# LPD-EPFL-ML/X-MAP

Hardware: AMD Instinct MI355X
Metric: item_sim_pairs_per_s (higher is better)
Workload: dtype f64

## Files before the change

include/xmap_hip.h:

```cpp
#ifndef XMAP_HIP_H
#define XMAP_HIP_H
#include <stdint.h>

#ifdef __cplusplus
extern "C" {
#endif

#define XMAP_OK 0
#define XMAP_ERR_HIP -1
#define XMAP_ERR_ARG -2
#define XMAP_ERR_OVERFLOW -3
#define XMAP_ERR_CAPACITY -4

#define XMAP_COSINE 0
#define XMAP_ADJUST_COSINE 1
#define XMAP_COSINE_EXACT 2

#define XMAP_TOPC 10

typedef struct xmap_ratings {
    int64_t n_users;
    int32_t n_items;
    int64_t nnz;
    const int64_t *user_ptr;
    const int32_t *user_item;
    const float *user_rating;
    const int64_t *user_time;
    const int64_t *item_ptr;
    const int32_t *item_user;
    const float *item_rating;
    const int32_t *prefix_cls;
    const int32_t *suffix_cls;
    const uint32_t *contains_mask;
    const uint8_t *flags;
} xmap_ratings;

const char *xmap_last_error(void);
int xmap_version(void);

int xmap_trim(void);
int xmap_debug_arena(void *stream, int64_t *live, int64_t *reserved);
int xmap_debug_arena_call(void *stream, int64_t bytes, int fail);

int xmap_exclusive_scan_i64(void *stream, const int64_t *in, int64_t *out, int64_t n, int64_t *h_total);
int xmap_exclusive_scan_i32_to_i64(void *stream, const int32_t *in, int64_t *out, int64_t n, int64_t *h_total);


int xmap_build_csc(void *stream, int64_t n_users, int32_t n_items, int64_t nnz, const int64_t *user_ptr,
                   const int32_t *user_item, const float *user_rating, int32_t *cnt ,
                   int64_t *item_ptr , int32_t *item_user , float *item_rating );

int xmap_user_stats(void *stream, const xmap_ratings *R, double *u_avg, double *u_norm2);

int xmap_item_stats(void *stream, const xmap_ratings *R, const double *u_avg, double *info ,
                    double *norms ,
                    int32_t *ua_item , int32_t *ia_user ,
                    int32_t item_lo, int32_t item_hi );

#ifdef XMAP_CROSSCHECK
int xmap_sim_plan(void *stream, const xmap_ratings *R, int32_t slot_target, int32_t *Q, int64_t *W, int64_t *unit_ptr,
                  int64_t *h_n_units, int64_t *h_contrib);
int xmap_sim_units(void *stream, int32_t n_items, const int32_t *Q, const int64_t *unit_ptr,
                   int32_t *unit_item , int32_t *unit_q );

int xmap_sim_count(void *stream, const xmap_ratings *R, int method, int cap, const double *u_avg,
                   const double *info, const int32_t *ua_item, const int32_t *ia_user, const int32_t *Q,
                   const int32_t *unit_item, const int32_t *unit_q, int64_t unit_lo, int64_t unit_hi,
                   int32_t *unit_cnt , int64_t *d_counters , int64_t *h_counters );
int xmap_sim_fill(void *stream, const xmap_ratings *R, int method, int cap, const double *u_avg,
                  const double *info, const int32_t *ua_item, const int32_t *ia_user, const int32_t *Q,
                  const int32_t *unit_item, const int32_t *unit_q, int64_t unit_lo, int64_t unit_hi,
                  const int64_t *unit_off , int32_t *col, double *sim, int32_t *mutu, int32_t *nij);

int xmap_sim_row_ptr(void *stream, int32_t n_items, const int64_t *unit_ptr, const int64_t *unit_off ,
                     int64_t *row_ptr );
#endif

int xmap_sim2_layout(void *stream, const xmap_ratings *R, const double *info, int32_t ch_min, int32_t *hist ,
                     int64_t *pre , int32_t *ctl , int32_t *hid , int32_t *hlist ,
                     uint64_t *ub_key , void *ub ,
                     void *rc ,
                     uint64_t *Wp ,
                     int32_t dups , int32_t *h_ctl );
int xmap_sim2_plan(void *stream, const xmap_ratings *R, int32_t slot_target, const void *rc, const int64_t *pre,
                   const int32_t *hid, const int32_t *ctl, int32_t *Q, int32_t *C, uint8_t *small ,
                   uint64_t *Wp , int32_t *Qcat , int64_t *uq_ptr ,
                   int64_t *uc_ptr , int32_t dups, int64_t *h_counts );
int xmap_sim2_units(void *stream, int32_t n_items, const int64_t *item_ptr, const int32_t *Qcat, const int64_t *uq_ptr,
                    int32_t *uq_item, int32_t *uq_q , const int32_t *C, const int64_t *uc_ptr, int32_t *uc_item,
                    int32_t *uc_c);
int xmap_sim2_pairs(void *stream, const xmap_ratings *R, int method, int cap, const double *u_avg, const double *norms,
                    const void *rc, const void *ub, const int32_t *Q,
                    const uint8_t *small, const int32_t *uq_item, const int32_t *uq_q, const int64_t *cls_ptr ,
                    int64_t unit_lo, int64_t unit_hi, const int32_t *hid,
                    const int32_t *hlist, const int32_t *ctl, const int32_t *C, const int64_t *uc_ptr,
                    const int32_t *uc_item, const int32_t *uc_c, int32_t n_heavy_units, int32_t n_heavy, int phases,
                    double *hp_hi, double *hp_lo, int32_t *hp_cnt, int32_t *hp_mut, int64_t coo_cap, int32_t *coo_i,
                    int32_t *coo_j, double *coo_sim, int32_t *coo_mutu, int32_t *coo_nij,
                    double *coo_ls , int32_t *rowcnt,
                    int32_t *rowcnt_h , int64_t *d_shards ,
                    int64_t *d_counters ,
                    int32_t *mircnt );
int xmap_sim2_scatter(void *stream, int32_t n_items, int64_t n_coo, const int32_t *coo_i, const int32_t *coo_j,
                      const double *coo_sim, const int32_t *coo_mutu, const int32_t *coo_nij, const double *coo_ls ,
                      const int64_t *row_ptr, int32_t *fill , const int32_t *hid, const int32_t *hlist,
                      int32_t *col, double *sim, int32_t *mutu, int32_t *nij, double *ls );
int xmap_sim3_layout(void *stream, const xmap_ratings *R, int64_t *item_ptr ,
                     const double *rating64 , int32_t ch_min, int32_t phases, int32_t stats_lo, int32_t stats_hi,
                     int32_t *cnt ,
                     double *u_avg , double *u_norm , int32_t *hist ,
                     int64_t *pre , int32_t *ctl , int32_t *hid , int32_t *hlist ,
                     uint64_t *ub_key , void *ub , void *srec ,
                     void *bufA , void *bufB , void *rc ,
                     uint64_t *Wp , double *info , double *norms , int32_t *h_ctl );
int xmap_sim3_plan(void *stream, const xmap_ratings *R, int32_t slot_target, const int64_t *pre, const int32_t *hid,
                   const int32_t *ctl, int32_t *Q, int32_t *C, uint8_t *small, uint64_t *Wp, int32_t *Qcat ,
                   int64_t *uq_ptr , int64_t *uc_ptr , int32_t dups, int32_t *uq_item, int32_t *uq_q ,
                   int32_t *uc_item, int32_t *uc_c, int64_t cap_light, int64_t cap_heavy, int64_t *h_out );
int xmap_sim3_mircount(void *stream, int32_t n_items, int64_t coo_cap, const int32_t *coo_i, const int32_t *coo_j,
                       const int64_t *d_shards , int64_t n_pairs, int32_t skip_self, void *scratch, int32_t *mir );
int xmap_sim3_mirror(void *stream, int32_t n_items, int64_t coo_cap, const int32_t *coo_i, const int32_t *coo_j,
                     const double *coo_sim, const int32_t *coo_mutu, const int32_t *coo_nij,
                     const int64_t *d_shards ,
                     int64_t n_pairs, const int32_t *own , const int32_t *mir , int32_t *tot ,
                     int64_t *row_ptr , int64_t *mptr , int32_t *fill ,
                     void *bufA , void *bufB , int32_t *col,
                     double *sim, int32_t *mutu, int32_t *nij, const double *coo_aux , double *aux ,
                     int32_t row_lo, int32_t row_hi );

int xmap_sim2_pack_pairs(void *stream, int64_t n_coo, const int32_t *coo_i, const int32_t *coo_j, const double *coo_sim,
                         const int32_t *coo_mutu, const int32_t *coo_nij, int64_t *rec , int64_t *h_count);
int xmap_sim2_unpack_pairs(void *stream, int64_t n, const int64_t *rec , int32_t *coo_i, int32_t *coo_j, double *coo_sim,
                           int32_t *coo_mutu, int32_t *coo_nij);
int xmap_item_partials(void *stream, const xmap_ratings *R, const double *u_avg, double *partial );
int xmap_item_merge(void *stream, int32_t n_items, int32_t n_parts, const double *parts , double *info ,
                    double *norms );
int xmap_sim2_pack_partials(void *stream, int64_t n_coo, const int32_t *coo_i, const int32_t *coo_j, const double *coo_hi,
                            const double *coo_lo, const int32_t *coo_mutu, const int32_t *coo_nij, int64_t *rec ,
                            int64_t *h_count);
int xmap_sim2_sort_partials(void *stream, int64_t n, const int64_t *rec , int64_t *rec_sorted , int32_t n_items,
                            int32_t n_owners );
int xmap_sim2_merge_partials(void *stream, int method, int cap, int32_t n_items, int64_t n, const int64_t *rec_sorted,
                             const double *norms , int32_t *coo_i, int32_t *coo_j, double *coo_sim, int32_t *coo_mutu,
                             int32_t *coo_nij, int32_t *rowcnt , int64_t *h_counts );



typedef struct xmap_sim {
    int32_t n_items;
    const int64_t *row_ptr;
    const int32_t *col;
    const double *sim;
    const int32_t *mutu;
    const int32_t *nij;
    const double *info;
    const double *frac;
} xmap_sim;

int xmap_bridge_flags(void *stream, const xmap_sim *S, const int32_t *prefix_cls, uint8_t *bb);

int xmap_knn_classify(void *stream, const xmap_sim *S, int top_k, const uint8_t *bb, const int32_t *suffix_cls,
                      const uint32_t *contains_mask, uint8_t *cls, int32_t *kcnt ,
                      int32_t *kcol , double *kval ,
                      int32_t row_lo, int32_t row_hi );

int xmap_knn_thresholds(void *stream, int32_t n_items, int top_k, const int32_t *kcnt, const int32_t *kcol, const double *kval,
                        void *thr );
int xmap_reverse_count(void *stream, const xmap_sim *S, int mode, int top_k, const uint8_t *bb, const uint8_t *cls,
                       const int32_t *kcnt, const int32_t *kcol, const double *kval, const int32_t *suffix_cls,
// ... 112 lines not shown
int xmap_rec_select(void *stream, int32_t n_items, const int64_t *row_ptr, const int32_t *col, const double *sim,
                    const double *ls, int32_t keep, int32_t *out_cnt, int32_t *out_col, double *out_sim, double *out_ls);

int xmap_predict(void *stream, int64_t n_test, const int32_t *test_user, const int32_t *test_item, const int64_t *nb_ptr,
                 const int32_t *nb_item, const double *nb_sim, const int64_t *rt_ptr, const int32_t *rt_user, const double *rt_rating,
                 const double *rt_time, const double *item_avg, const double *wtab, int32_t n_w, double *out_plain,
                 double *out_decay, int32_t *status);

int xmap_rec_profiles(void *stream, int64_t n_users, int64_t n_rows, int64_t n_target_rows, const int64_t *off_t, const int64_t *off_m,
                      const int32_t *user, const int32_t *item, const double *rating, const int64_t *time, int64_t *prof_ptr,
                      int32_t *prof_item, double *prof_rating, int64_t *prof_time);
int xmap_predict_rows(void *stream, int64_t n_test, const int32_t *test_user, const int32_t *test_item, int64_t n_users,
                      int32_t n_items, int32_t keep, const int32_t *nb_cnt, const int32_t *nb_col, const double *nb_sim,
                      const int64_t *prof_ptr, const int32_t *prof_item, const double *prof_rating, const int64_t *prof_time,
                      const double *item_avg, const double *wtab, int32_t n_w, double *out_plain, double *out_decay,
                      int32_t *status, int32_t *h_max_now);
int xmap_mae(void *stream, int64_t n_test, const int32_t *status, const double *real, const double *out_plain, const double *out_decay,
             double *mae );


int xmap_select_map(void *stream, int32_t n_items, int private_flag, const int32_t *n_cand, const int32_t *top_end,
                    const int32_t *picks , int32_t *n_top, int32_t *choice, int32_t *map_src2tgt);

int xmap_alterego_count(void *stream, const xmap_ratings *R, const int32_t *map_src2tgt, int32_t *cnt_t, int32_t *cnt_m,
                        int64_t *d_profiles );
int xmap_alterego_fill(void *stream, const xmap_ratings *R, const int32_t *map_src2tgt, const int64_t *off_t,
                       const int64_t *off_m, int64_t n_t_total, int32_t *out_user, int32_t *out_item,
                       double *out_rating, int64_t *out_time);

typedef struct xmap_ctx xmap_ctx;

typedef struct xmap_feed xmap_feed;
int xmap_feed_text(const char *text, int64_t len, int32_t year_from, int32_t year_to, const char *label, int32_t min_ratings,
                   xmap_feed **out);
int xmap_feed_texts(int32_t n_parts, const char *const *texts, const int64_t *lens, const char *const *labels, int32_t year_from,
                    int32_t year_to, int32_t min_ratings, xmap_feed **out);
int xmap_feed_merge(const xmap_feed *a, const xmap_feed *b, xmap_feed **out);
int xmap_feed_sizes(const xmap_feed *f, int64_t *sizes );
int xmap_feed_arrays(const xmap_feed *f, int64_t *user_ptr, int32_t *item, double *rating, double *when, int32_t *prefix_cls,
                     int32_t *suffix_cls, uint32_t *contains_mask, uint8_t *flags);
int xmap_feed_ids(const xmap_feed *f, int32_t which, char *bytes, int64_t *offsets);
void xmap_feed_free(xmap_feed *f);
int xmap_ctx_upload_feed(xmap_ctx *ctx, const xmap_feed *f);
int xmap_feed_format(int64_t n_users, const int64_t *user_ptr, const int32_t *item, const float *rating, const int64_t *when,
                     const char *uid_fmt, const char *iid_fmt, const int64_t *item_number, int32_t item_lo, int32_t item_hi,
                     char *out, int64_t cap, int64_t *written);

int xmap_ctx_create(int device, xmap_ctx **out);
void xmap_ctx_destroy(xmap_ctx *ctx);
int xmap_ctx_upload_ratings(xmap_ctx *ctx, int64_t n_users, int32_t n_items, const int64_t *user_ptr, const int32_t *item,
                            const float *rating, const int64_t *time, const int32_t *prefix_cls, const int32_t *suffix_cls,
                            const uint32_t *contains_mask, const uint8_t *flags);
int xmap_ctx_item_sim(xmap_ctx *ctx, int method, int cap, int64_t *n_kept, int64_t *n_evaluated);
int xmap_ctx_sim_download(xmap_ctx *ctx, int64_t *row_ptr, int32_t *col, double *sim, int32_t *mutu, int32_t *nij, double *info,
                          double *user_avg);
int xmap_ctx_extend(xmap_ctx *ctx, int top_k, int64_t *n_out, int64_t *n_paths);
int xmap_ctx_ext_download(xmap_ctx *ctx, int32_t *n_cand, int32_t *top_end, double *top_val);
int xmap_ctx_ext_lists(xmap_ctx *ctx, int64_t *xs_off, int32_t *xs_end, double *xs_val);
int xmap_ctx_candidates(xmap_ctx *ctx, int32_t *n_top);
int xmap_ctx_generate(xmap_ctx *ctx, int private_flag, const int32_t *picks, int32_t *choice, int64_t *n_rows,
                      int64_t *n_target_rows);
int xmap_ctx_gen_download(xmap_ctx *ctx, int32_t *user, int32_t *item, double *rating, int64_t *time);
int xmap_ctx_rec_sim(xmap_ctx *ctx, int cap, int64_t *n_pairs);
int xmap_ctx_rec_profiles_download(xmap_ctx *ctx, int64_t *prof_ptr, int32_t *prof_item, double *prof_rating, int64_t *prof_time);
int xmap_ctx_rec_download(xmap_ctx *ctx, int64_t *row_ptr, int32_t *col, double *sim, double *ls, int32_t *nij, double *item_avg,
                          double *item_norm);
int xmap_ctx_rec_select(xmap_ctx *ctx, int keep);
int xmap_ctx_rec_set_neighbors(xmap_ctx *ctx, int keep, const int32_t *cnt, const int32_t *col, const double *sim);
int xmap_ctx_rec_neighbors_download(xmap_ctx *ctx, int32_t *cnt, int32_t *col, double *sim, double *ls);
int xmap_ctx_predict(xmap_ctx *ctx, int64_t n_test, const int32_t *test_user, const int32_t *test_item, const double *test_rating,
                     const double *wtab, int32_t n_w, double *out_plain, double *out_decay, int32_t *status, double *mae,
                     int32_t *max_now);

#ifdef __cplusplus
}
#endif
#endif
```

profiles/lds_atomic.hip:

```cpp
#include <hip/hip_runtime.h>
#include <stdio.h>
#define CK(x) do { hipError_t e_ = (x); if (e_ != hipSuccess) { printf("%s -> %s\n", #x, hipGetErrorString(e_)); return 1; } } while (0)
__device__ __forceinline__ unsigned long long mix(unsigned long long z) {
    z += 0x9E3779B97F4A7C15ull; z = (z ^ (z >> 30)) * 0xBF58476D1CE4E5B9ull; z = (z ^ (z >> 27)) * 0x94D049BB133111EBull;
    return z ^ (z >> 31);
}
template <int MODE>
__global__ __launch_bounds__(1024) void k(double *out, int steps, int n_slots) {
    extern __shared__ double tab[];
    for (int i = threadIdx.x; i < n_slots * 4; i += 1024) tab[i] = 0.0;
    __syncthreads();
    unsigned long long s = mix(blockIdx.x * 1024ull + threadIdx.x);
    double chk = 0.0;
    for (int it = 0; it < steps; it++) {
        s = mix(s);
        const int slot = (int)(s % (unsigned)n_slots);
        const double v = (double)(s & 1023) * 0.001, c = 0.5;
        double *a = tab + slot * 4;
        if (MODE == 0) {
            const double o = atomicAdd(a, v);
            const double sum = o + v, bb = sum - o;
            const double err = (o - (sum - bb)) + (v - bb);
            atomicAdd(a + 1, err);
            const double o2 = atomicAdd(a + 2, c);
            const double sum2 = o2 + c, bb2 = sum2 - o2;
            const double err2 = (o2 - (sum2 - bb2)) + (c - bb2);
            atomicAdd(a + 3, err2);
        } else {
            double h = a[0], l = a[1], h2 = a[2], l2 = a[3];
            double sum = h + v, bb = sum - h; double e = (h - (sum - bb)) + (v - bb); e += l; double hh = sum + e; l = e - (hh - sum); h = hh;
            double sum2 = h2 + c, bb2 = sum2 - h2; double e2 = (h2 - (sum2 - bb2)) + (c - bb2); e2 += l2; double hh2 = sum2 + e2; l2 = e2 - (hh2 - sum2); h2 = hh2;
            a[0] = h; a[1] = l; a[2] = h2; a[3] = l2;
        }
    }
    __syncthreads();
    for (int i = threadIdx.x; i < n_slots * 4; i += 1024) chk += tab[i];
    if (chk == 12345.678) out[0] = chk;
}
int main() {
    double *out; CK(hipMalloc(&out, 8));
    hipEvent_t e0, e1; CK(hipEventCreate(&e0)); CK(hipEventCreate(&e1));
    const int steps = 4096, blocks = 256 * 4;
    for (int n_slots : {512, 2048, 4096}) {
        const size_t lds = (size_t)n_slots * 32;
        CK(hipFuncSetAttribute((const void *)k<0>, hipFuncAttributeMaxDynamicSharedMemorySize, (int)lds));
        CK(hipFuncSetAttribute((const void *)k<1>, hipFuncAttributeMaxDynamicSharedMemorySize, (int)lds));
        for (int mode = 0; mode < 2; mode++)
            for (int rep = 0; rep < 2; rep++) {
                CK(hipEventRecord(e0));
                if (mode == 0) k<0><<<blocks, 1024, lds>>>(out, steps, n_slots); else k<1><<<blocks, 1024, lds>>>(out, steps, n_slots);
                CK(hipEventRecord(e1)); CK(hipEventSynchronize(e1));
                float ms; CK(hipEventElapsedTime(&ms, e0, e1));
                const double n = (double)blocks * 1024 * steps;
                if (rep) printf("slots %5d mode %d (%s): %7.2f ms  %.3e updates/s\n", n_slots, mode, mode ? "plain 32-B RMW" : "4 atomics + 2 two-sums", ms, n / (ms * 1e-3));
            }
    }
    return 0;
}
```

x-map_amd/csrc/api.hip:

```cpp
#include <math.h>
#include <stdlib.h>
#include <vector>

#include "common.h"

namespace xmap {

struct Pool {
    std::vector<void *> ptrs;
    void release() {
        for (void *p : ptrs) (void)hipFree(p);
        ptrs.clear();
    }
};

}

using namespace xmap;

struct xmap_ctx {
    int device = 0;
    hipStream_t st = nullptr;
    Pool p_ratings, p_sim, p_ext, p_gen, p_rows;
    xmap_ratings R;
    bool have_ratings = false;
    bool plain_exact = true;
    bool have_sim = false;
    xmap_sim S;
    double *u_avg = nullptr, *u_norm = nullptr, *info = nullptr;
    int64_t n_kept = 0, n_eval = 0, n_contrib = 0;
    int64_t half_contrib = 0;
    bool have_ext = false;
    int top_k = 0;
    xmap_ext_tables T;
    xmap_path_units Un;
    int32_t *n_cand = nullptr, *top_end = nullptr;
    double *top_val = nullptr;
    int64_t n_out = 0, n_paths = 0;
    double *acc = nullptr, *hacc = nullptr;
    int32_t *touched = nullptr, *htouched = nullptr;
    int64_t acc_slots = 0, acc_len = 0, hacc_rows = 0, hacc_len = 0;
    int32_t n_slots = 0;
    int32_t fast_div = 0;
    bool have_gen = false;
    int32_t *g_user = nullptr, *g_item = nullptr;
    double *g_rating = nullptr;
    int64_t *g_time = nullptr;
    int64_t n_rows = 0, n_target_rows = 0;
    int64_t *g_off_t = nullptr, *g_off_m = nullptr;
    Pool p_rec, p_nb;
    bool have_rec = false, have_nb = false;
    int64_t *pf_ptr = nullptr, *pf_time = nullptr;
    int32_t *pf_item = nullptr;
    double *pf_rating = nullptr;
    int64_t *rs_row_ptr = nullptr;
    int32_t *rs_col = nullptr, *rs_nij = nullptr;
    double *rs_sim = nullptr, *rs_ls = nullptr, *rs_avg = nullptr, *rs_norm = nullptr;
    int64_t rec_pairs = 0;
    int keep = 0;
    int32_t *nb_cnt = nullptr, *nb_col = nullptr;
    double *nb_sim = nullptr, *nb_ls = nullptr;
};

namespace xmap {

template <typename T>
static int dalloc(Pool &pool, T **out, size_t n, hipStream_t st, bool zero = false) {
    void *p = nullptr;
    const size_t bytes = sizeof(T) * (n ? n : 1);
    XM_HIP(hipMalloc(&p, bytes));
    pool.ptrs.push_back(p);
    if (zero) XM_HIP(hipMemsetAsync(p, 0, bytes, st));
    *out = (T *)p;
    return XMAP_OK;
}
#define XM_TRY(call) do { int rc_ = (call); if (rc_) return rc_; } while (0)
#define XM_ALLOC(pool, ptr, n) XM_TRY(dalloc(pool, &(ptr), (size_t)(n), c->st))
#define XM_ALLOCZ(pool, ptr, n) XM_TRY(dalloc(pool, &(ptr), (size_t)(n), c->st, true))

// ... 148 lines not shown
    R.n_users = n_users; R.n_items = n_items; R.nnz = nnz;
    c->half_contrib = 0;
    for (int64_t u = 0; u < n_users; u++) { const int64_t d = user_ptr[u + 1] - user_ptr[u]; c->half_contrib += d * (d - 1) / 2; }
    int64_t *d_ptr, *d_time, *d_iptr;
    int32_t *d_item, *d_iuser, *d_pre, *d_suf;
    float *d_rating, *d_irating;
    uint32_t *d_mask;
    uint8_t *d_flags;
    XM_TRY(h2d(c->p_ratings, &d_ptr, user_ptr, (size_t)n_users + 1, c->st));
    XM_TRY(h2d(c->p_ratings, &d_item, item, (size_t)nnz, c->st));
    XM_TRY(h2d(c->p_ratings, &d_rating, rating, (size_t)nnz, c->st));
    XM_TRY(h2d(c->p_ratings, &d_time, time, (size_t)nnz, c->st));
    XM_TRY(h2d(c->p_ratings, &d_pre, prefix_cls, (size_t)n_items, c->st));
    XM_TRY(h2d(c->p_ratings, &d_suf, suffix_cls, (size_t)n_items, c->st));
    XM_TRY(h2d(c->p_ratings, &d_mask, contains_mask, (size_t)n_items, c->st));
    XM_TRY(h2d(c->p_ratings, &d_flags, flags, (size_t)n_items, c->st));
    XM_ALLOCZ(c->p_ratings, d_iptr, n_items + 1);
    XM_ALLOCZ(c->p_ratings, d_iuser, nnz);
    XM_ALLOCZ(c->p_ratings, d_irating, nnz);
    R.user_ptr = d_ptr; R.user_item = d_item; R.user_rating = d_rating; R.user_time = d_time;
    R.item_ptr = d_iptr; R.item_user = d_iuser; R.item_rating = d_irating;
    R.prefix_cls = d_pre; R.suffix_cls = d_suf; R.contains_mask = d_mask; R.flags = d_flags;
    c->plain_exact = plain_sums_exact(n_users, nnz, rating);
    XM_HIP(hipStreamSynchronize(c->st));
    c->have_ratings = true;
    return XMAP_OK;
}

int xmap_ctx_item_sim(xmap_ctx *c, int method, int cap, int64_t *n_kept, int64_t *n_evaluated) {
    XM_ARG(c && c->have_ratings && (method == XMAP_COSINE || method == XMAP_ADJUST_COSINE) && cap > 0);
    XM_HIP(hipSetDevice(c->device));
    drop_tail(c);
    c->p_gen.release(); c->p_ext.release(); c->p_sim.release();
    c->have_sim = c->have_ext = c->have_gen = false;
    xmap_ratings &R = c->R;
    const int I = R.n_items;
    const int64_t U = R.n_users, nnz = R.nnz;
    const int pair_method = (method == XMAP_COSINE && !c->plain_exact) ? XMAP_COSINE_EXACT : method;
    Pool tmp;
    struct Guard { Pool &p; ~Guard() { p.release(); } } guard{tmp};
#define T_ALLOC(ptr, n) XM_TRY(dalloc(tmp, &(ptr), (size_t)(n), c->st))
#define T_ALLOCZ(ptr, n) XM_TRY(dalloc(tmp, &(ptr), (size_t)(n), c->st, true))
    int32_t *cnt;
    T_ALLOC(cnt, I);
    double *norms;
    XM_ALLOC(c->p_sim, c->u_avg, U);
    XM_ALLOC(c->p_sim, c->u_norm, U);
    XM_ALLOCZ(c->p_sim, c->info, (size_t)I * 4);
    T_ALLOCZ(norms, (size_t)2 * I);
    int32_t *hist, *ctl, *hid, *hlist;
    int64_t *pre;
    uint64_t *ub_key, *ub, *rcrec, *Wp, *srec, *buf_a, *buf_b;
    const size_t n1 = (size_t)(nnz ? nnz : 1);
    T_ALLOC(hist, U + 2); T_ALLOC(pre, U + 3); T_ALLOC(ctl, 4); T_ALLOC(hid, I); T_ALLOCZ(hlist, 1024);
    T_ALLOC(ub_key, n1); T_ALLOC(ub, n1); T_ALLOC(rcrec, 2 * n1); T_ALLOC(Wp, I);
    T_ALLOC(srec, 2 * n1); T_ALLOC(buf_a, 2 * n1); T_ALLOC(buf_b, 2 * n1);
    const int ch_min = 2048;
    XM_TRY(xmap_sim3_layout(c->st, &R, (int64_t *)R.item_ptr, nullptr, ch_min, 1 | 2 | 4, 0, I, cnt, c->u_avg, c->u_norm, hist, pre, ctl,
                            hid, hlist, ub_key, ub, srec, buf_a, buf_b, rcrec, Wp, c->info, norms, nullptr));
    const int64_t half_contrib = c->half_contrib;
    int32_t *Q, *Cc, *Qcat, *uq_item = nullptr, *uq_q = nullptr, *uc_item = nullptr, *uc_c = nullptr;
    uint8_t *small;
    int64_t *uq_ptr, *uc_ptr;
    T_ALLOCZ(Q, I); T_ALLOCZ(Cc, I); T_ALLOCZ(small, I); T_ALLOC(Qcat, (size_t)5 * (I ? I : 1)); T_ALLOCZ(uq_ptr, (size_t)5 * I + 1);
    T_ALLOCZ(uc_ptr, I + 1);
    int slot_target = 768;
    double coo_slack = 1.0;
    int64_t hc[10];
    int64_t n_light = 0, n_hu = 0;
    int n_heavy = 0;
    auto plan = [&](int target) -> int {
        const int64_t cap_light = half_contrib / target + I + 1, cap_heavy = nnz / ch_min + 1025;
        T_ALLOC(uq_item, cap_light); T_ALLOC(uq_q, 4 * cap_light); T_ALLOC(uc_item, cap_heavy); T_ALLOC(uc_c, cap_heavy);
        XM_TRY(xmap_sim3_plan(c->st, &R, target, pre, hid, ctl, Q, Cc, small, Wp, Qcat, uq_ptr, uc_ptr, 0, uq_item, uq_q, uc_item, uc_c,
                              cap_light, cap_heavy, hc));
        n_light = hc[0]; n_hu = hc[1]; n_heavy = (int)hc[9];
        return XMAP_OK;
    };
    XM_TRY(plan(slot_target));
    int32_t *coo_i = nullptr, *coo_j = nullptr, *coo_mutu = nullptr, *coo_nij = nullptr, *own = nullptr, *mir = nullptr;
    double *coo_sim = nullptr;
    int64_t *d_shards = nullptr;
    int64_t cap_coo = 0, n = 0, n_unordered = 0;
    for (;;) {
        cap_coo = ((int64_t)((double)(half_contrib > 0 ? half_contrib : 1) * coo_slack) / 4096 + 1100) * 4096;
        double *hp_hi, *hp_lo;
        int32_t *hp_cnt, *hp_mut, *rowcnt_h;
        int64_t *d_cnt;
        T_ALLOC(coo_i, cap_coo); T_ALLOC(coo_j, cap_coo); T_ALLOC(coo_sim, cap_coo); T_ALLOC(coo_mutu, cap_coo); T_ALLOC(coo_nij, cap_coo);
        T_ALLOC(own, I); T_ALLOC(mir, I);
        const size_t hp = (size_t)(n_hu ? n_hu : 1) * 1024;
        T_ALLOC(hp_hi, hp); T_ALLOC(hp_lo, hp); T_ALLOC(hp_cnt, hp); T_ALLOC(hp_mut, hp);
        T_ALLOCZ(d_cnt, 6); T_ALLOC(d_shards, 2 * 4096); T_ALLOC(rowcnt_h, 64 * 1024);
        XM_TRY(xmap_sim2_pairs(c->st, &R, pair_method, cap, c->u_avg, norms, rcrec, ub, Q, small, uq_item, uq_q, hc + 2, 0, n_light, hid, hlist,
                               ctl, Cc, uc_ptr, uc_item, uc_c, (int32_t)n_hu, n_heavy, 8 | 1 | 2 | 4 | 16 | 64 | 128, hp_hi, hp_lo, hp_cnt,
                               hp_mut, cap_coo, coo_i, coo_j, coo_sim, coo_mutu, coo_nij, nullptr, own, rowcnt_h, d_shards, d_cnt, mir));
        int64_t h_cnt[6];
        XM_TRY(d2h(h_cnt, d_cnt, 6, c->st));
        XM_HIP(hipStreamSynchronize(c->st));
        if (h_cnt[2]) {
            if (slot_target <= 32) { set_error("pair-table overflow"); return XMAP_ERR_OVERFLOW; }
            slot_target /= 2;
            XM_TRY(plan(slot_target));
            continue;
        }
        if (h_cnt[3]) {
            if (coo_slack > 64) { set_error("half-COO overflow"); return XMAP_ERR_CAPACITY; }
            coo_slack *= 2;
            continue;
        }
        n = h_cnt[4]; n_unordered = h_cnt[5];
        break;
    }
    int64_t *row_ptr, *mptr;
    XM_ALLOCZ(c->p_sim, row_ptr, I + 1);
    T_ALLOCZ(mptr, I + 1);
    const int64_t kept = 2 * n;
    int32_t *col, *mutu, *nij, *fill, *tot;
    double *sim;
    uint64_t *mir_a, *mir_b;
    XM_ALLOC(c->p_sim, col, kept); XM_ALLOC(c->p_sim, sim, kept); XM_ALLOC(c->p_sim, mutu, kept); XM_ALLOC(c->p_sim, nij, kept);
    T_ALLOC(fill, I); T_ALLOC(tot, I); T_ALLOC(mir_a, (size_t)3 * (n ? n : 1)); T_ALLOC(mir_b, (size_t)3 * (n ? n : 1));
    XM_TRY(xmap_sim3_mircount(c->st, I, cap_coo, coo_i, coo_j, d_shards, n, 0, mir_a, mir));
    XM_TRY(xmap_sim3_mirror(c->st, I, cap_coo, coo_i, coo_j, coo_sim, coo_mutu, coo_nij, d_shards, n, own, mir, tot, row_ptr, mptr, fill,
                            mir_a, mir_b, col, sim, mutu, nij, nullptr, nullptr, 0, I));
    XM_HIP(hipStreamSynchronize(c->st));
    c->S.n_items = I; c->S.row_ptr = row_ptr; c->S.col = col; c->S.sim = sim; c->S.mutu = mutu; c->S.nij = nij; c->S.info = c->info;
    c->S.frac = nullptr;
    c->n_kept = kept; c->n_eval = 2 * n_unordered; c->n_contrib = 2 * half_contrib;
    c->have_sim = true;
    if (n_kept) *n_kept = kept;
    if (n_evaluated) *n_evaluated = c->n_eval;
    return XMAP_OK;
#undef T_ALLOC
#undef T_ALLOCZ
}

int xmap_ctx_sim_download(xmap_ctx *c, int64_t *row_ptr, int32_t *col, double *sim, int32_t *mutu, int32_t *nij, double *info,
                          double *user_avg) {
    XM_ARG(c && c->have_sim);
    XM_HIP(hipSetDevice(c->device));
    const int I = c->R.n_items;
    if (row_ptr) XM_TRY(d2h(row_ptr, c->S.row_ptr, (size_t)I + 1, c->st));
    if (col) XM_TRY(d2h(col, c->S.col, (size_t)c->n_kept, c->st));
    if (sim) XM_TRY(d2h(sim, c->S.sim, (size_t)c->n_kept, c->st));
    if (mutu) XM_TRY(d2h(mutu, c->S.mutu, (size_t)c->n_kept, c->st));
    if (nij) XM_TRY(d2h(nij, c->S.nij, (size_t)c->n_kept, c->st));
    if (info) XM_TRY(d2h(info, (const double *)c->info, (size_t)I * 4, c->st));
    if (user_avg) XM_TRY(d2h(user_avg, (const double *)c->u_avg, (size_t)c->R.n_users, c->st));
    XM_HIP(hipStreamSynchronize(c->st));
    return XMAP_OK;
}

int xmap_ctx_extend(xmap_ctx *c, int top_k, int64_t *n_out, int64_t *n_paths) {
    XM_ARG(c && c->have_sim && top_k >= 1);
    XM_HIP(hipSetDevice(c->device));
    drop_tail(c);
    c->p_gen.release(); c->p_ext.release();
    c->have_ext = c->have_gen = false;
    const int I = c->R.n_items, k = top_k;
    c->top_k = k;
    xmap_ext_tables &T = c->T;
    memset(&T, 0, sizeof(T));
    T.n_items = I; T.top_k = k; T.flags = c->R.flags;
    XM_ALLOCZ(c->p_ext, c->n_cand, I);
    XM_ALLOC(c->p_ext, c->top_end, (size_t)I * XMAP_TOPC);
    XM_ALLOCZ(c->p_ext, c->top_val, (size_t)I * XMAP_TOPC);
    c->n_out = c->n_paths = 0;
    if (I == 0) { c->have_ext = true; if (n_out) *n_out = 0; if (n_paths) *n_paths = 0; return XMAP_OK; }
    uint8_t *bb, *cls;
    int32_t *kcnt, *kcol;
    double *kval;
    XM_ALLOCZ(c->p_ext, bb, I); XM_ALLOC(c->p_ext, cls, I); XM_ALLOC(c->p_ext, kcnt, (size_t)I * 2);
    XM_ALLOC(c->p_ext, kcol, (size_t)I * 2 * k); XM_ALLOC(c->p_ext, kval, (size_t)I * 2 * k * 3);
    XM_TRY(xmap_bridge_flags(c->st, &c->S, c->R.prefix_cls, bb));
    XM_TRY(xmap_knn_classify(c->st, &c->S, k, bb, c->R.suffix_cls, c->R.contains_mask, cls, kcnt, kcol, kval, 0, I));
    T.cls = cls; T.kcnt = kcnt; T.kcol = kcol; T.kval = kval;
    XM_TRY(xmap_edge_ranges(c->st, &c->S, &c->fast_div));
    double *thr;
    int32_t *long_rows;
    XM_ALLOC(c->p_ext, thr, (size_t)I * 4);
    XM_ALLOC(c->p_ext, long_rows, I + 1);
    uint8_t *eflag;
    XM_ALLOC(c->p_ext, eflag, (size_t)(c->n_kept > 0 ? c->n_kept : 1));
    XM_TRY(xmap_knn_thresholds(c->st, I, k, kcnt, kcol, kval, thr));
    const uint8_t *dummy;
    int32_t *cnt_att, *cnt_rnn;
    XM_ALLOCZ(c->p_ext, cnt_att, I);
// ... 151 lines not shown
    XM_HIP(hipSetDevice(c->device));
    const size_t n = (size_t)c->n_rows;
    if (user) XM_TRY(d2h(user, (const int32_t *)c->g_user, n, c->st));
    if (item) XM_TRY(d2h(item, (const int32_t *)c->g_item, n, c->st));
    if (rating) XM_TRY(d2h(rating, (const double *)c->g_rating, n, c->st));
    if (time) XM_TRY(d2h(time, (const int64_t *)c->g_time, n, c->st));
    XM_HIP(hipStreamSynchronize(c->st));
    return XMAP_OK;
}


int xmap_ctx_rec_sim(xmap_ctx *c, int cap, int64_t *n_pairs) {
    XM_ARG(c && c->have_gen && cap > 0);
    XM_HIP(hipSetDevice(c->device));
    drop_tail(c);
    const int I = c->R.n_items;
    const int64_t U = c->R.n_users, nnz = c->n_rows;
    XM_ARG(nnz < 2147483647ll);
    const size_t n1 = (size_t)(nnz ? nnz : 1), i1 = (size_t)(I ? I : 1);
    XM_ALLOCZ(c->p_rec, c->pf_ptr, U + 1);
    XM_ALLOC(c->p_rec, c->pf_item, n1); XM_ALLOC(c->p_rec, c->pf_rating, n1); XM_ALLOC(c->p_rec, c->pf_time, n1);
    XM_TRY(xmap_rec_profiles(c->st, U, nnz, c->n_target_rows, c->g_off_t, c->g_off_m, c->g_user, c->g_item, c->g_rating, c->g_time,
                             c->pf_ptr, c->pf_item, c->pf_rating, c->pf_time));
    XM_ALLOCZ(c->p_rec, c->rs_row_ptr, I + 1);
    XM_ALLOCZ(c->p_rec, c->rs_avg, i1); XM_ALLOCZ(c->p_rec, c->rs_norm, i1);
    c->rec_pairs = 0;
    if (I == 0 || nnz == 0) {
        XM_HIP(hipStreamSynchronize(c->st));
        c->have_rec = true;
        if (n_pairs) *n_pairs = 0;
        return XMAP_OK;
    }
    std::vector<int64_t> h_ptr((size_t)U + 1);
    XM_TRY(d2h(h_ptr.data(), (const int64_t *)c->pf_ptr, (size_t)U + 1, c->st));
    XM_HIP(hipStreamSynchronize(c->st));
    int64_t half_contrib = 0;
    for (int64_t u = 0; u < U; u++) { const int64_t d = h_ptr[u + 1] - h_ptr[u]; half_contrib += d * (d - 1) / 2; }
    Pool tmp;
    struct Guard { Pool &p; ~Guard() { p.release(); } } guard{tmp};
#define T_ALLOC(ptr, n) XM_TRY(dalloc(tmp, &(ptr), (size_t)(n), c->st))
#define T_ALLOCZ(ptr, n) XM_TRY(dalloc(tmp, &(ptr), (size_t)(n), c->st, true))
    xmap_ratings P = c->R;
    float *f_dummy, *f_irating;
    int64_t *item_ptr;
    int32_t *i_user;
    T_ALLOCZ(f_dummy, n1); T_ALLOCZ(f_irating, n1); T_ALLOCZ(item_ptr, I + 1); T_ALLOCZ(i_user, n1);
    P.nnz = nnz; P.user_ptr = c->pf_ptr; P.user_item = c->pf_item; P.user_rating = f_dummy; P.user_time = c->pf_time;
    P.item_ptr = item_ptr; P.item_user = i_user; P.item_rating = f_irating;
    int32_t *cnt, *hist, *ctl, *hid, *hlist;
    int64_t *pre;
    uint64_t *ub_key, *ub, *rcrec, *Wp, *srec, *buf_a, *buf_b;
    double *u_avg, *info, *norms;
    T_ALLOC(cnt, i1); T_ALLOCZ(u_avg, U ? U : 1); T_ALLOCZ(info, i1 * 4); T_ALLOCZ(norms, 2 * i1);
    T_ALLOC(hist, U + 2); T_ALLOC(pre, U + 3); T_ALLOC(ctl, 4); T_ALLOC(hid, i1); T_ALLOCZ(hlist, 1024);
    T_ALLOC(ub_key, n1); T_ALLOC(ub, 2 * n1); T_ALLOC(rcrec, 2 * n1); T_ALLOC(Wp, i1);
    T_ALLOC(srec, 3 * n1); T_ALLOC(buf_a, 3 * n1); T_ALLOC(buf_b, 3 * n1);
    const int ch_min = (int)((U + 2 > 64) ? U + 2 : 64);
    XM_TRY(xmap_sim3_layout(c->st, &P, item_ptr, c->pf_rating, ch_min, 1 | 2 | 4, 0, I, cnt, u_avg, nullptr, hist, pre, ctl, hid, hlist,
                            ub_key, ub, srec, buf_a, buf_b, rcrec, Wp, info, norms, nullptr));
    int32_t *Q, *Cc, *Qcat, *uq_item = nullptr, *uq_q = nullptr, *uc_item = nullptr, *uc_c = nullptr;
    uint8_t *small;
    int64_t *uq_ptr, *uc_ptr;
    T_ALLOCZ(Q, i1); T_ALLOCZ(Cc, i1); T_ALLOCZ(small, i1); T_ALLOC(Qcat, 5 * i1); T_ALLOCZ(uq_ptr, (size_t)5 * I + 1);
    T_ALLOCZ(uc_ptr, I + 1);
    int slot_target = 768;
    double coo_slack = 1.0;
    int64_t hc[10];
    int64_t n_light = 0;
    auto plan = [&](int target) -> int {
        const int64_t cap_light = half_contrib / target + I + 1, cap_heavy = nnz / ch_min + 1025;
        T_ALLOC(uq_item, cap_light); T_ALLOC(uq_q, 4 * cap_light); T_ALLOC(uc_item, cap_heavy); T_ALLOC(uc_c, cap_heavy);
        XM_TRY(xmap_sim3_plan(c->st, &P, target, pre, hid, ctl, Q, Cc, small, Wp, Qcat, uq_ptr, uc_ptr, 1, uq_item, uq_q, uc_item, uc_c,
                              cap_light, cap_heavy, hc));
        n_light = hc[0];
        return XMAP_OK;
    };
    XM_TRY(plan(slot_target));
    int32_t *coo_i = nullptr, *coo_j = nullptr, *coo_mutu = nullptr, *coo_nij = nullptr, *own = nullptr, *mir = nullptr;
    double *coo_sim = nullptr, *coo_ls = nullptr;
    int64_t *d_shards = nullptr;
    int64_t cap_coo = 0, n = 0;
    for (;;) {
        cap_coo = ((int64_t)((double)(half_contrib > 0 ? half_contrib : 1) * coo_slack) / 4096 + 1100) * 4096;
        double *hp_hi, *hp_lo;
        int32_t *hp_cnt, *hp_mut, *rowcnt_h;
        int64_t *d_cnt;
        T_ALLOC(coo_i, cap_coo); T_ALLOC(coo_j, cap_coo); T_ALLOC(coo_sim, cap_coo); T_ALLOC(coo_mutu, cap_coo); T_ALLOC(coo_nij, cap_coo);
        T_ALLOC(coo_ls, cap_coo); T_ALLOC(own, i1); T_ALLOC(mir, i1);
        T_ALLOC(hp_hi, 1024); T_ALLOC(hp_lo, 1024); T_ALLOC(hp_cnt, 1024); T_ALLOC(hp_mut, 1024);
        T_ALLOCZ(d_cnt, 6); T_ALLOC(d_shards, 2 * 4096); T_ALLOC(rowcnt_h, 64 * 1024);
        XM_TRY(xmap_sim2_pairs(c->st, &P, XMAP_ADJUST_COSINE, cap, u_avg, norms, rcrec, ub, Q, small, uq_item, uq_q, hc + 2, 0, n_light, hid,
                               hlist, ctl, Cc, uc_ptr, uc_item, uc_c, 0, 0, 8 | 2 | 16 | 64 | 128, hp_hi, hp_lo, hp_cnt, hp_mut, cap_coo,
                               coo_i, coo_j, coo_sim, coo_mutu, coo_nij, coo_ls, own, rowcnt_h, d_shards, d_cnt, mir));
        int64_t h_cnt[6];
        XM_TRY(d2h(h_cnt, d_cnt, 6, c->st));
        XM_HIP(hipStreamSynchronize(c->st));
        if (h_cnt[2]) {
            if (slot_target <= 32) { set_error("pair-table overflow"); return XMAP_ERR_OVERFLOW; }
            slot_target /= 2;
            XM_TRY(plan(slot_target));
            continue;
        }
        if (h_cnt[3]) {
            if (coo_slack > 64) { set_error("half-COO overflow"); return XMAP_ERR_CAPACITY; }
            coo_slack *= 2;
            continue;
        }
        n = h_cnt[4];
        break;
    }
    int64_t *mptr;
    T_ALLOCZ(mptr, I + 1);
    const size_t kept_max = (size_t)(n ? 2 * n : 1), nn = (size_t)(n ? n : 1);
    int32_t *mutu, *fill, *tot;
    uint64_t *mir_a, *mir_b;
    XM_ALLOC(c->p_rec, c->rs_col, kept_max); XM_ALLOC(c->p_rec, c->rs_sim, kept_max); XM_ALLOC(c->p_rec, c->rs_nij, kept_max);
    XM_ALLOC(c->p_rec, c->rs_ls, kept_max);
    T_ALLOC(mutu, kept_max); T_ALLOC(fill, i1); T_ALLOC(tot, i1); T_ALLOC(mir_a, 4 * nn); T_ALLOC(mir_b, 4 * nn);
    XM_TRY(xmap_sim3_mircount(c->st, I, cap_coo, coo_i, coo_j, d_shards, n, 1, mir_a, mir));
    XM_TRY(xmap_sim3_mirror(c->st, I, cap_coo, coo_i, coo_j, coo_sim, coo_mutu, coo_nij, d_shards, n, own, mir, tot, c->rs_row_ptr, mptr, fill,
                            mir_a, mir_b, c->rs_col, c->rs_sim, mutu, c->rs_nij, coo_ls, c->rs_ls, 0, I));
    XM_HIP(hipMemcpy2DAsync(c->rs_avg, sizeof(double), info, 4 * sizeof(double), sizeof(double), (size_t)I, hipMemcpyDeviceToDevice, c->st));
    XM_HIP(hipMemcpyAsync(c->rs_norm, norms + I, sizeof(double) * (size_t)I, hipMemcpyDeviceToDevice, c->st));
    int64_t kept = 0;
    XM_TRY(d2h(&kept, (const int64_t *)(c->rs_row_ptr + I), 1, c->st));
    XM_HIP(hipStreamSynchronize(c->st));
    c->rec_pairs = kept;
    c->have_rec = true;
    if (n_pairs) *n_pairs = kept;
    return XMAP_OK;
#undef T_ALLOC
#undef T_ALLOCZ
}

int xmap_ctx_rec_profiles_download(xmap_ctx *c, int64_t *prof_ptr, int32_t *prof_item, double *prof_rating, int64_t *prof_time) {
    XM_ARG(c && c->have_rec);
    XM_HIP(hipSetDevice(c->device));
    const size_t n = (size_t)c->n_rows;
    if (prof_ptr) XM_TRY(d2h(prof_ptr, (const int64_t *)c->pf_ptr, (size_t)c->R.n_users + 1, c->st));
    if (prof_item) XM_TRY(d2h(prof_item, (const int32_t *)c->pf_item, n, c->st));
    if (prof_rating) XM_TRY(d2h(prof_rating, (const double *)c->pf_rating, n, c->st));
    if (prof_time) XM_TRY(d2h(prof_time, (const int64_t *)c->pf_time, n, c->st));
    XM_HIP(hipStreamSynchronize(c->st));
    return XMAP_OK;
}

// ... 105 lines not shown
```

x-map_amd/csrc/common.h:

```cpp
#pragma once
#if defined(__HIP_DEVICE_COMPILE__) && !defined(__gfx950__)
#error "libxmap_hip is written for gfx950 (MI355X): build with --offload-arch=gfx950"
#endif
#include <hip/hip_runtime.h>
#include <stdint.h>
#include <stdio.h>
#include <string.h>

#include "../../include/xmap_hip.h"

namespace xmap {

void set_error(const char *fmt, ...);

#define XM_HIP(call)                                                                         \
    do {                                                                                     \
        hipError_t e_ = (call);                                                              \
        if (e_ != hipSuccess) {                                                              \
            xmap::set_error("%s:%d %s -> %s", __FILE__, __LINE__, #call, hipGetErrorString(e_)); \
            return XMAP_ERR_HIP;                                                             \
        }                                                                                    \
    } while (0)

#define XM_LAUNCH_CHECK() XM_HIP(hipGetLastError())

#define XM_ARG(cond)                                                        \
    do {                                                                    \
        if (!(cond)) {                                                      \
            xmap::set_error("%s:%d bad argument: %s", __FILE__, __LINE__, #cond); \
            return XMAP_ERR_ARG;                                            \
        }                                                                   \
    } while (0)

hipError_t xm_malloc_async(void **p, size_t bytes, hipStream_t st);
hipError_t xm_free_async(void *p, hipStream_t st);
struct XmScope {
    int dev; hipStream_t st; size_t live0; bool ok;
    explicit XmScope(hipStream_t st);
    ~XmScope();
    XmScope(const XmScope &) = delete;
    XmScope &operator=(const XmScope &) = delete;
};
#define XM_SCOPE(stream) xmap::XmScope xm_scope_((hipStream_t)(stream))
int radix_sort_pairs(hipStream_t st, unsigned long long *keys, int *vals, unsigned long long *keys_tmp, int *vals_tmp, long long n,
                     int bits);

constexpr int WAVE = 64;

__device__ __forceinline__ int lane_id() { return threadIdx.x & 63; }

__device__ __forceinline__ int rl32(int v, int l) { return __builtin_amdgcn_readlane(v, l); }
__device__ __forceinline__ float rlf(float v, int l) { return __int_as_float(rl32(__float_as_int(v), l)); }
__device__ __forceinline__ long long rl64(long long v, int l) {
    int lo = rl32((int)(v & 0xffffffffll), l), hi = rl32((int)(v >> 32), l);
    return ((long long)hi << 32) | (unsigned int)lo;
}
__device__ __forceinline__ double rld(double v, int l) {
    return __longlong_as_double(rl64(__double_as_longlong(v), l));
}
__device__ __forceinline__ int uniform(int v) { return __builtin_amdgcn_readfirstlane(v); }

__device__ __forceinline__ unsigned long long lanemask_lt() {
    return (1ull << lane_id()) - 1ull;
}

__device__ __forceinline__ double wave_sum(double v) {
#pragma unroll
    for (int m = 32; m >= 1; m >>= 1) v += __shfl_xor(v, m, 64);
    return v;
}
__device__ __forceinline__ long long wave_sum_ll(long long v) {
#pragma unroll
    for (int m = 32; m >= 1; m >>= 1) v += __shfl_xor(v, m, 64);
    return v;
}

__device__ __forceinline__ void dd_add(double &hi, double &lo, double x) {
    double s = hi + x;
    double bb = s - hi;
    double e = (hi - (s - bb)) + (x - bb);
    e += lo;
    double h2 = s + e;
    lo = e - (h2 - s);
    hi = h2;
}

template <int G>
__device__ __forceinline__ void dd_reduce(double &hi, double &lo) {
#pragma unroll
    for (int m = G / 2; m >= 1; m >>= 1) {
        double oh = __shfl_down(hi, m, G), ol = __shfl_down(lo, m, G);
        dd_add(hi, lo, oh);
        dd_add(hi, lo, ol);
    }
}

__device__ __forceinline__ uint32_t mix32(uint32_t h) {
    h ^= h >> 16; h *= 0x85EBCA6Bu; h ^= h >> 13; h *= 0xC2B2AE35u; h ^= h >> 16;
// ... 5 lines not shown
```

x-map_amd/csrc/stage_a.hip:

```cpp
#include "common.h"
#include "item_stats.h"

namespace xmap {

#ifdef XMAP_CROSSCHECK
constexpr int A_THREADS = 64;
constexpr int A_WAVES = A_THREADS / 64;
constexpr int LOG_SLOTS = 10;
constexpr int SLOTS = 1 << LOG_SLOTS;
constexpr uint32_t EMPTY = 0xFFFFFFFFu;
#endif

__global__ __launch_bounds__(256) void k_user_stats(long long U, const long long *ptr, const float *rating,
                                                    double *avg, double *norm2) {
    long long u = (long long)blockIdx.x * blockDim.x + threadIdx.x;
    if (u >= U) return;
    long long a = ptr[u], b = ptr[u + 1];
    double s = 0.0, q = 0.0;
    for (long long e = a; e < b; e++) {
        double r = (double)rating[e];
        s += r;
        q += r * r;
    }
    avg[u] = (b > a) ? s / (double)(b - a) : 0.0;
    norm2[u] = sqrt(q);
}

constexpr int CSC_SLOTS = 4096;
constexpr int CSC_CHUNK = 8192;
constexpr int CSC_USERS = 512;
__device__ __forceinline__ int csc_slot(int it) { return (int)(mix32((uint32_t)it) & (CSC_SLOTS - 1)); }

__global__ __launch_bounds__(256) void k_csc_count(long long nnz, const int *uitem, int *cnt) {
    __shared__ int tag[CSC_SLOTS], loc[CSC_SLOTS];
    for (int t = threadIdx.x; t < CSC_SLOTS; t += 256) { tag[t] = -1; loc[t] = 0; }
    __syncthreads();
    const long long e0 = (long long)blockIdx.x * CSC_CHUNK;
    for (int q = threadIdx.x; q < CSC_CHUNK; q += 256) {
        const long long e = e0 + q;
        if (e >= nnz) break;
        const int it = uitem[e];
        const int sl = csc_slot(it);
        const int old = atomicCAS(&tag[sl], -1, it);
        if (old == -1 || old == it) atomicAdd(&loc[sl], 1); else atomicAdd(&cnt[it], 1);
    }
    __syncthreads();
    for (int t = threadIdx.x; t < CSC_SLOTS; t += 256)
        if (loc[t]) atomicAdd(&cnt[tag[t]], loc[t]);
}

__global__ __launch_bounds__(256) void k_csc_fill(long long U, const long long *uptr, const int *uitem, const float *urating,
                                                  const long long *iptr, int *cur, int *iuser, float *irating) {
    __shared__ int tag[CSC_SLOTS], loc[CSC_SLOTS], base[CSC_SLOTS];
    for (int t = threadIdx.x; t < CSC_SLOTS; t += 256) { tag[t] = -1; loc[t] = 0; }
    __syncthreads();
    const long long u0 = (long long)blockIdx.x * CSC_USERS;
    const long long u1 = min(U, u0 + CSC_USERS);
    const int w = threadIdx.x >> 6, lane = lane_id();
    for (long long u = u0 + w; u < u1; u += 4)
        for (long long e = uptr[u] + lane; e < uptr[u + 1]; e += 64) {
            const int it = uitem[e];
            const int sl = csc_slot(it);
            const int old = atomicCAS(&tag[sl], -1, it);
            if (old == -1 || old == it) atomicAdd(&loc[sl], 1);
        }
    __syncthreads();
    for (int t = threadIdx.x; t < CSC_SLOTS; t += 256) {
        if (loc[t]) base[t] = atomicAdd(&cur[tag[t]], loc[t]);
        loc[t] = 0;
    }
    __syncthreads();
    for (long long u = u0 + w; u < u1; u += 4)
        for (long long e = uptr[u] + lane; e < uptr[u + 1]; e += 64) {
            const int it = uitem[e];
            const int sl = csc_slot(it);
            const int off = (tag[sl] == it) ? base[sl] + atomicAdd(&loc[sl], 1) : atomicAdd(&cur[it], 1);
            const long long p = iptr[it] + off;
            iuser[p] = (int)u;
// ... 259 lines not shown
        out += c;
        kept += c;
    }
    if (!WRITE && lane == 0) {
        A.unit_cnt[unit] = kept;
        atomicAdd(&A.counters[0], (unsigned long long)kept);
        atomicAdd(&A.counters[1], (unsigned long long)evald);
    }
    if (__ballot(ovf) && lane == 0) atomicOr(&A.counters[2], 1ull);
}

static int launch_pair(hipStream_t st, int method, bool write, const PairArgs &A) {
    long long n = A.unit_hi - A.unit_lo;
    if (n <= 0) return XMAP_OK;
    dim3 grid((unsigned)((n + A_WAVES - 1) / A_WAVES)), block(A_THREADS);
    if (method == XMAP_COSINE) {
        if (write) k_pair_sim<XMAP_COSINE, true><<<grid, block, 0, st>>>(A);
        else k_pair_sim<XMAP_COSINE, false><<<grid, block, 0, st>>>(A);
    } else if (method == XMAP_COSINE_EXACT) {
        if (write) k_pair_sim<XMAP_COSINE_EXACT, true><<<grid, block, 0, st>>>(A);
        else k_pair_sim<XMAP_COSINE_EXACT, false><<<grid, block, 0, st>>>(A);
    } else {
        if (write) k_pair_sim<XMAP_ADJUST_COSINE, true><<<grid, block, 0, st>>>(A);
        else k_pair_sim<XMAP_ADJUST_COSINE, false><<<grid, block, 0, st>>>(A);
    }
    XM_LAUNCH_CHECK();
    return XMAP_OK;
}

static PairArgs make_args(const xmap_ratings *R, int cap, const double *u_avg, const double *info, const int32_t *ua_item,
                          const int32_t *ia_user, const int32_t *Q, const int32_t *unit_item, const int32_t *unit_q,
                          int64_t lo, int64_t hi) {
    PairArgs A;
    memset(&A, 0, sizeof(A));
    A.uptr = (const long long *)R->user_ptr;
    A.ua_item = ua_item;
    A.urating = R->user_rating;
    A.iptr = (const long long *)R->item_ptr;
    A.ia_user = ia_user;
    A.irating = R->item_rating;
    A.u_avg = u_avg;
    A.info = info;
    A.Q = Q;
    A.unit_item = unit_item;
    A.unit_q = unit_q;
    A.unit_lo = lo;
    A.unit_hi = hi;
    A.cap = cap;
    return A;
}

#endif

}

using namespace xmap;

extern "C" {

int xmap_build_csc(void *stream, int64_t n_users, int32_t n_items, int64_t nnz, const int64_t *user_ptr,
                   const int32_t *user_item, const float *user_rating, int32_t *cnt ,
                   int64_t *item_ptr , int32_t *item_user, float *item_rating) {
    XM_ARG(user_ptr && cnt && item_ptr && (nnz == 0 || (user_item && user_rating && item_user && item_rating)));
    XM_ARG(nnz < 0x7fffffffLL);
    hipStream_t st = (hipStream_t)stream;
    XM_HIP(hipMemsetAsync(cnt, 0, sizeof(int32_t) * (size_t)(n_items > 0 ? n_items : 1), st));
    if (nnz > 0) {
        k_csc_count<<<dim3((unsigned)((nnz + CSC_CHUNK - 1) / CSC_CHUNK)), dim3(256), 0, st>>>(nnz, user_item, cnt);
        XM_LAUNCH_CHECK();
    }
    int rc = xmap_exclusive_scan_i32_to_i64(stream, cnt, item_ptr, n_items, nullptr);
    if (rc) return rc;
    XM_HIP(hipMemsetAsync(cnt, 0, sizeof(int32_t) * (size_t)(n_items > 0 ? n_items : 1), st));
    if (nnz > 0) {
        k_csc_fill<<<dim3((unsigned)((n_users + CSC_USERS - 1) / CSC_USERS)), dim3(256), 0, st>>>(
            n_users, (const long long *)user_ptr, user_item, user_rating, (const long long *)item_ptr, cnt, item_user,
            item_rating);
        XM_LAUNCH_CHECK();
    }
    return XMAP_OK;
}

int xmap_user_stats(void *stream, const xmap_ratings *R, double *u_avg, double *u_norm2) {
    XM_ARG(R && u_avg && u_norm2);
    if (R->n_users == 0) return XMAP_OK;
    hipStream_t st = (hipStream_t)stream;
    k_user_stats<<<dim3((unsigned)((R->n_users + 255) / 256)), dim3(256), 0, st>>>(
        R->n_users, (const long long *)R->user_ptr, R->user_rating, u_avg, u_norm2);
    XM_LAUNCH_CHECK();
    return XMAP_OK;
}

int xmap_item_stats(void *stream, const xmap_ratings *R, const double *u_avg, double *info, double *norms,
                    int32_t *ua_item, int32_t *ia_user, int32_t item_lo, int32_t item_hi) {
    XM_ARG(R && u_avg && info && ((ua_item != nullptr) == (ia_user != nullptr)));
    XM_ARG(R->nnz < 0x7fffffffLL && item_lo >= 0 && item_lo <= item_hi && item_hi <= R->n_items);
    hipStream_t st = (hipStream_t)stream;
    if (item_hi > item_lo) {
        k_item_stats<<<dim3((unsigned)((item_hi - item_lo + 15) / 16)), dim3(256), 0, st>>>(
            R->n_items, item_lo, item_hi, (const long long *)R->item_ptr, R->item_user, R->item_rating, u_avg, info, norms, ia_user);
        XM_LAUNCH_CHECK();
    }
#ifdef XMAP_CROSSCHECK
    if (R->nnz > 0 && ua_item) {
        k_pack_user_side<<<dim3((unsigned)((R->nnz + 255) / 256)), dim3(256), 0, st>>>(
            R->nnz, R->user_item, R->user_rating, info, ua_item);
        XM_LAUNCH_CHECK();
    }
#else
    XM_ARG(ua_item == nullptr);
#endif
    return XMAP_OK;
}

int xmap_item_partials(void *stream, const xmap_ratings *R, const double *u_avg, double *partial ) {
    XM_ARG(R && u_avg && partial && R->nnz < 0x7fffffffLL);
    hipStream_t st = (hipStream_t)stream;
    if (R->n_items > 0) {
        k_item_stats<<<dim3((unsigned)((R->n_items + 15) / 16)), dim3(256), 0, st>>>(
            R->n_items, 0, R->n_items, (const long long *)R->item_ptr, R->item_user, R->item_rating, u_avg, nullptr, nullptr, nullptr,
            partial);
        XM_LAUNCH_CHECK();
    }
    return XMAP_OK;
}

int xmap_item_merge(void *stream, int32_t n_items, int32_t n_parts, const double *parts, double *info, double *norms) {
    XM_ARG(parts && info && norms && n_items >= 0 && n_parts >= 1);
    if (n_items > 0) {
        k_item_merge<<<dim3((unsigned)((n_items + 255) / 256)), dim3(256), 0, (hipStream_t)stream>>>(n_items, n_parts, parts, info, norms);
        XM_LAUNCH_CHECK();
    }
    return XMAP_OK;
}

#ifdef XMAP_CROSSCHECK
int xmap_sim_plan(void *stream, const xmap_ratings *R, int32_t slot_target, int32_t *Q, int64_t *W, int64_t *unit_ptr,
                  int64_t *h_n_units, int64_t *h_contrib) {
    XM_SCOPE(stream);
    XM_ARG(R && Q && W && unit_ptr && slot_target > 0 && slot_target <= SLOTS);
    hipStream_t st = (hipStream_t)stream;
    unsigned long long *d_contrib = nullptr;
    XM_HIP(xm_malloc_async((void **)&d_contrib, sizeof(unsigned long long), st));
// ... 86 lines not shown
```

x-map_amd/csrc/stage_a2.hip:

```cpp
#include <type_traits>

#include "common.h"
#include "item_stats.h"
#include "tilesort.h"

namespace xmap {

constexpr int T_LOG_SLOTS = 10;
constexpr int T_SLOTS = 1 << T_LOG_SLOTS;
constexpr int HMAX = 1024;
constexpr uint32_t T_EMPTY = 0xFFFFFFFFu;
constexpr int SMALL_BOUND = 96;
constexpr int MID_BOUND = 384;

constexpr int N_CLASSES = 5;
constexpr int WIDE_MIN = 2048;
__host__ __device__ __forceinline__ int class_rank(int cls) {
    return cls == 4 ? 0 : (cls == 0 ? 1 : (cls == 2 ? 2 : (cls == 3 ? 3 : 4)));
}

__device__ __forceinline__ unsigned long long wkey(int n, int item) {
    return ((unsigned long long)(unsigned)n << 32) | (unsigned)item;
}

// ... 203 lines not shown
    small[i] = (uint8_t)cls;
    Wp[i] = (unsigned long long)w;
    Qcat[(size_t)class_rank(cls) * I + i] = q;
}

__global__ __launch_bounds__(256) void k_plan2(int I, const long long *iptr, const RaterRec *rc, const long long *pre,
                                               int HB, const int *hid, const int *CH, int target, int dups, int *Q, int *C,
                                               uint8_t *small, unsigned long long *Wp, int *Qcat) {
    const int i = blockIdx.x * blockDim.x + threadIdx.x;
    if (i >= I) return;
    plan_item(i, (long long)Wp[i], I, iptr, pre, HB, hid, CH, target, dups, Q, C, small, Wp, Qcat);
}

__global__ __launch_bounds__(256) void k_fill_units2(int I, const long long *iptr, const int *Qcat, const long long *uq_ptr,
                                                     int *uq_item, int *uq_q, const int *C, const long long *uc_ptr, int *uc_item,
                                                     int *uc_c, long long cap_light, long long cap_heavy) {
    const long long x = (long long)blockIdx.x * blockDim.x + threadIdx.x;
    if (x >= (long long)N_CLASSES * I) return;
    const int i = (int)(x % I);
    long long b = uq_ptr[x];
    const int nq = Qcat[x];
    if (nq > 0) {
        const int p0 = (int)iptr[i], p1 = (int)iptr[i + 1];
        for (int k = 0; k < nq && b + k < cap_light; k++) {
            uq_item[b + k] = i;
            ((int4 *)uq_q)[b + k] = make_int4(k, p0, p1, nq);
        }
    }
    if (x >= I) return;
    b = uc_ptr[i];
    for (int k = 0; k < C[i] && b + k < cap_heavy; k++) { uc_item[b + k] = i; uc_c[b + k] = k; }
}

struct TriArgs {
    const long long *iptr;
    const RaterRec *rc;
    const int2 *ub;
    const double *u_avg; const double *nrm;
    int cap;
    const int *Q; const uint8_t *small; const int *uq_item; const int *uq_q; long long unit_lo, unit_hi;
    const int *hid; const int *hlist; const int *CH; const int *uc_item; const int *uc_c;
    const long long *uc_ptr; const int *C;
    double *hp_hi; double *hp_lo; int *hp_cnt; int *hp_mut;
    long long shard_cap;
    unsigned long long *shard_cur;
    unsigned long long *shard_occ;
    int *coo_i; int *coo_j; double *coo_sim; int *coo_mutu; int *coo_nij;
    double *coo_aux;
    int *rowcnt;
    int *mircnt;
    int *rowcnt_h;
    unsigned long long *counters;
    int heavy_mod, heavy_rem;
    int raw;
};

template <int METHOD>
__device__ __forceinline__ bool finish_pair(const TriArgs &A, int i, int j, int n, int m, double dot, double &simv) {
    const double np = A.nrm[i] * A.nrm[j];
    const double cs = (np != 0.0) ? 1.0 * dot / np : 0.0;
    const int mn = n < A.cap ? n : A.cap;
    simv = 1.0 * cs * (double)mn / (double)A.cap;
    return (simv != 0.0) && (m != 0);
}

constexpr int COO_SHARDS = 4096;


template <typename Fin, typename Park, typename Get, typename Aux>
__device__ __forceinline__ void append_pairs(const TriArgs &A, int i, int s_begin, int n_slots, Fin fin, Park park, Get get,
                                             Aux aux) {
    const int lane = lane_id();
    const int shard = (blockIdx.x * (blockDim.x >> 6) + uniform((int)(threadIdx.x >> 6))) & (COO_SHARDS - 1);
    int kept = 0, occ = 0;
    for (int s0 = s_begin; s0 < n_slots; s0 += 64) {
        int j, n, m; double sv; bool o;
        bool keep = fin(s0 + lane, j, n, m, sv, o);
        park(s0 + lane, o, keep, sv);
        kept += __popcll(__ballot(keep));
        occ += __popcll(__ballot(o));
    }
    if (lane == 0 && occ) atomicAdd(&A.shard_occ[shard], (unsigned long long)occ);
    if (!kept) return;
    unsigned long long base = 0;
    if (lane == 0) {
        base = atomicAdd(&A.shard_cur[shard], (unsigned long long)kept);
        atomicAdd(&A.rowcnt[i], kept);
    }
    base = ((unsigned long long)(unsigned)rl32((int)(base >> 32), 0) << 32) | (unsigned)rl32((int)(base & 0xffffffffull), 0);
    if ((long long)(base + kept) > A.shard_cap) {
        if (lane == 0) atomicOr(&A.counters[3], 1ull);
        return;
    }
    base += (unsigned long long)shard * (unsigned long long)A.shard_cap;
    for (int s0 = s_begin; s0 < n_slots; s0 += 64) {
        int j, n, m; double sv;
        bool keep = get(s0 + lane, j, n, m, sv);
        unsigned long long km = __ballot(keep);
        if (keep) {
            long long p = (long long)base + __popcll(km & lanemask_lt());
            A.coo_i[p] = i; A.coo_j[p] = j;
            A.coo_sim[p] = sv; A.coo_mutu[p] = m; A.coo_nij[p] = n;
            if (A.coo_aux) A.coo_aux[p] = aux(s0 + lane);
        }
        base += __popcll(km);
    }
}

__global__ __launch_bounds__(256) void k_shard_sums(const unsigned long long *shards, unsigned long long *counters) {
    unsigned long long a = 0ull, b = 0ull;
    for (int s = threadIdx.x; s < COO_SHARDS; s += 256) { a += shards[s]; b += shards[COO_SHARDS + s]; }
    a = (unsigned long long)wave_sum_ll((long long)a);
    b = (unsigned long long)wave_sum_ll((long long)b);
    if (lane_id() == 0) { atomicAdd(&counters[4], a); atomicAdd(&counters[5], b); }
}


__device__ __forceinline__ double weighted(double cs, int n, int cap) {
    const int mn = n < cap ? n : cap;
    return 1.0 * cs * (double)mn / (double)cap;
}
__device__ __forceinline__ unsigned long long ls_key(double d) {
    return (d != d) ? 0x7ff8000000000000ull : (unsigned long long)__double_as_longlong(d);
}

static_assert(std::is_standard_layout<TriArgs>::value, "KARG() addresses TriArgs fields by offsetof");
#define KARG(field) (*(decltype(TriArgs::field) const volatile __attribute__((address_space(4))) *)( \
    (const char __attribute__((address_space(4))) *)__builtin_amdgcn_kernarg_segment_ptr() + offsetof(TriArgs, field)))
template <int METHOD, int LOG_SLOTS, int NW, bool LS>
__global__ __launch_bounds__(64 * NW, (LOG_SLOTS == 7 && !LS) ? 8 : 1) void k_pair_tri(TriArgs A) {
    constexpr int SLOTS_ = 1 << LOG_SLOTS;
    constexpr bool ADJ = METHOD == XMAP_ADJUST_COSINE;
    using RT = typename std::conditional<LS, double, float>::type;
    using CM = typename std::conditional<NW == 16 || LS, unsigned long long, unsigned>::type;
    constexpr int MSH = (NW == 16 || LS) ? 32 : 16;
    constexpr CM NMASK = (CM)(((CM)1 << MSH) - 1);
    constexpr uint32_t LOCKBIT = 0x80000000u;
    __shared__ uint32_t key[SLOTS_];
    __shared__ CM cm[SLOTS_];
    __shared__ double dot[SLOTS_];
    __shared__ double dlo[ADJ ? SLOTS_ : 1];
    __shared__ unsigned short claim[ADJ && NW == 1 ? SLOTS_ : 1];
    __shared__ double s_ny[LS ? SLOTS_ : 1];
    __shared__ unsigned long long s_ls[LS ? SLOTS_ : 1];
    __shared__ int s_ovf;
    static_assert(!LS || ADJ, "the local-sensitivity pass keeps the similarity in dlo[]");

    const int lane = lane_id();
    const long long unit = A.unit_lo + blockIdx.x;
    if (unit >= A.unit_hi) return;
    const int i = uniform(A.uq_item[unit]);
    const int4 ud = ((const int4 *)A.uq_q)[unit];
    const int q = uniform(ud.x), p0 = uniform(ud.y), p1 = uniform(ud.z), Qi = uniform(ud.w);
    const int w = uniform((int)uniform((int)(threadIdx.x >> 6)));
    for (int s = threadIdx.x; s < SLOTS_; s += 64 * NW) {
        key[s] = T_EMPTY; cm[s] = (CM)0; dot[s] = 0.0;
        if (ADJ) dlo[s] = 0.0;
    }
    if (NW > 1) {
        if (threadIdx.x == 0) s_ovf = 0;
        __syncthreads();
    }
    const double nx = A.nrm[i];
    int ovf = 0;

    constexpr int RB = (NW == 1 || NW == 16) ? 64 : 16;
    constexpr int WU = 2;
    struct RawRec { int e0, pw, usr; RT r; };
    auto rater = [&](int p) {
        const int pc = (lane < RB && p < p1) ? p : p0;
        RawRec o;
        if (LS) {
            const RaterRecWide rr = ((const RaterRecWide *)A.rc)[pc];
            o.e0 = rr.e0; o.pw = rr.pos_ge; o.r = (RT)rr.rating; o.usr = 0;
        } else {
            const RaterRec rr = A.rc[pc];
            o.e0 = rr.e0; o.pw = rr.pos_ge; o.r = (RT)rr.rating; o.usr = rr.user;
        }
        return o;
    };
    auto entry = [&](int e, int &jw_, RT &rj_) {
        if (LS) { const UbWide v = ((const UbWide *)A.ub)[e]; jw_ = v.item_ge; rj_ = (RT)v.rating; }
        else { const int2 v = A.ub[e]; jw_ = v.x; rj_ = (RT)__int_as_float(v.y); }
    };
    auto walk = [&](auto &&body) {
        int base = p0 + RB * w;
        if (base >= p1) return;
        RawRec cur = rater(base + lane);
        for (; base < p1; base += RB * NW) {
            RawRec nxt = cur;
            if (base + RB * NW < p1) nxt = rater(base + RB * NW + lane);
            const bool ok = lane < RB && base + lane < p1;
            const int e0 = cur.e0, pw = cur.pw, usr = cur.usr;
            const RT r = cur.r;
            const int len = ok ? (pw & 0x7fffffff) : 0;
            int end = len;
#pragma unroll
            for (int d = 1; d < RB; d <<= 1) { const int v = __shfl_up(end, d, 64); if (lane >= d) end += v; }
            const int total = rl32(end, RB - 1);
            const int start = end - len;
            for (int f0 = 0; f0 < total; f0 += 64 * WU) {
                int jw[WU]; RT rj[WU]; bool act[WU]; double ri[WU], a[WU]; unsigned gei[WU];
                int tt[WU], ee[WU], uu[WU];
#pragma unroll
                for (int u = 0; u < WU; u++) {
                    const int f = f0 + u * 64 + lane;
                    act[u] = f < total;
                    int t = 0;
#pragma unroll
                    for (int step = RB / 2; step >= 1; step >>= 1) { const int v = __shfl(end, t + step - 1, 64); if (v <= f) t += step; }
                    const int eb = __shfl(e0, t, 64), sb = __shfl(start, t, 64), ut = __shfl(usr, t, 64);
                    tt[u] = t;
                    ee[u] = act[u] ? eb + (f - sb) : 0;
                    uu[u] = act[u] ? ut : 0;
                }
#pragma unroll
                for (int u = 0; u < WU; u++) {
                    entry(ee[u], jw[u], rj[u]);
                    a[u] = 0.0;
                    if (ADJ && !LS) a[u] = A.u_avg[uu[u]];
                }
#pragma unroll
                for (int u = 0; u < WU; u++) {
                    const int pwt = __shfl(pw, tt[u], 64);
                    ri[u] = (double)__shfl(r, tt[u], 64);
                    gei[u] = ((unsigned)pwt) >> 31;
                }
#pragma unroll
                for (int u = 0; u < WU; u++) {
                    if (u && f0 + u * 64 >= total) continue;
                    const int j = jw[u] & 0x7fffffff;
                    bool ac = act[u];
                    if (ac && Qi > 1) ac = (int)__umulhi(mix32((uint32_t)j), (uint32_t)Qi) == q;
                    body(ac, j, jw[u], rj[u], ri[u], a[u], gei[u]);
                }
            }
            cur = nxt;
        }
    };

    walk([&](bool act, int j, int jw, RT rj, double ri, double a, unsigned gei) {
        uint32_t h = 0;
        if (act) {
            h = ((uint32_t)j * 0x9E3779B1u) >> (32 - LOG_SLOTS);
            int probes = 0;
            for (;;) {
                uint32_t prev = atomicCAS(&key[h], T_EMPTY, (uint32_t)j);
                if (prev == T_EMPTY || (prev & ~LOCKBIT) == (uint32_t)j) break;
                h = (h + 1) & (SLOTS_ - 1);
                if (++probes >= SLOTS_) { act = false; ovf = 1; break; }
            }
        }
        if (act) {
            const CM inc = (CM)1 | (((((unsigned)jw) >> 31) == gei) ? ((CM)1 << MSH) : (CM)0);
            atomicAdd(&cm[h], inc);
            if (METHOD == XMAP_COSINE) atomicAdd(&dot[h], (1.0 * ri) * (double)rj);
        }
        if (ADJ) {
            const double term = (ri - a) * ((double)rj - a);
            typedef __attribute__((address_space(3))) volatile double lds_vf64;
            typedef __attribute__((address_space(3))) volatile unsigned short lds_vu16;
            lds_vf64 *vhi = (lds_vf64 *)dot, *vlo = (lds_vf64 *)dlo;
            bool pending = act;
            if (NW == 1) {
                lds_vu16 *vclaim = (lds_vu16 *)claim;
                while (__ballot(pending)) {
                    if (pending) vclaim[h] = (unsigned short)lane;
                    if (pending && vclaim[h] == (unsigned short)lane) {
                        double hi = vhi[h], lo = vlo[h];
                        dd_add(hi, lo, term);
                        vhi[h] = hi; vlo[h] = lo;
                        pending = false;
                    }
                }
            } else {
                while (__ballot(pending)) {
                    if (pending && !(atomicOr(&key[h], LOCKBIT) & LOCKBIT)) {
                        double hi = vhi[h], lo = vlo[h];
                        dd_add(hi, lo, term);
                        vhi[h] = hi; vlo[h] = lo;
                        __threadfence_block();
                        atomicAnd(&key[h], ~LOCKBIT);
                        pending = false;
                    }
                }
            }
        }
    });
    if (NW > 1) {
        if (ovf) s_ovf = 1;
        __syncthreads();
        ovf = s_ovf;
    }
    if (__ballot(ovf)) {
        if (threadIdx.x == 0) atomicOr(&A.counters[2], 1ull);
        return;
    }
    if (LS) {
        const double nx = A.nrm[i];
        for (int s = threadIdx.x; s < SLOTS_; s += 64 * NW) {
            const uint32_t kj = key[s];
            if (kj == T_EMPTY) continue;
            int n = (int)(cm[s] & NMASK);
            double inner = dot[s];
            if ((int)kj == i) { n *= 2; inner *= 2.0; }
            const double ny = A.nrm[kj];
            const double np = nx * ny;
            cm[s] = (CM)(unsigned)n;
            dot[s] = inner;
            dlo[s] = weighted((np != 0.0) ? 1.0 * inner / np : 0.0, n, A.cap);
            s_ny[s] = ny;
            s_ls[s] = 0ull;
        }
        if (NW > 1) __syncthreads();
        walk([&](bool act, int j, int jw, RT rj, double ri, double a, unsigned gei) {
            if (!act) return;
            uint32_t h = ((uint32_t)j * 0x9E3779B1u) >> (32 - LOG_SLOTS);
            while (key[h] != (uint32_t)j) h = (h + 1) & (SLOTS_ - 1);
            const double inner = dot[h], sim = dlo[h], ny = s_ny[h];
            const int n = (int)cm[h];
            const double r0 = ri, r1 = (double)rj;
            const double rest = inner - r0 * r1;
            const double m1 = sqrt((nx * nx - r0 * r0) * (ny * ny));
            const double m2 = sqrt((nx * nx) * (ny * ny - r1 * r1));
            const double d1 = fabs(weighted((m1 != 0.0) ? 1.0 * rest / m1 : 0.0, n - 1, A.cap) - sim);
            const double d2 = fabs(weighted((m2 != 0.0) ? 1.0 * rest / m2 : 0.0, n - 1, A.cap) - sim);
            const unsigned long long k1 = ls_key(d1), k2 = ls_key(d2);
            atomicMax(&s_ls[h], k1 > k2 ? k1 : k2);
        });
        if (NW > 1) __syncthreads();
        append_pairs(A, i, w * (SLOTS_ / NW), (w + 1) * (SLOTS_ / NW),
            [&](int s, int &j, int &n, int &m, double &sv, bool &o) {
                const uint32_t kj = key[s];
                o = kj != T_EMPTY;
                if (!o) return false;
                j = (int)kj; n = (int)cm[s]; m = 0; sv = dlo[s];
                return true;
            },
            [&](int s, bool o, bool keep, double sv) {},
            [&](int s, int &j, int &n, int &m, double &sv) {
                const uint32_t kj = key[s];
                if (kj == T_EMPTY) return false;
                j = (int)kj; n = (int)cm[s]; m = 0; sv = dlo[s];
                return true;
            },
            [&](int s) { return __longlong_as_double((long long)s_ls[s]); });
        return;
    }
    const auto k_coo_i = KARG(coo_i);
    const auto k_coo_j = KARG(coo_j);
    const auto k_coo_sim = KARG(coo_sim);
    const auto k_coo_mutu = KARG(coo_mutu);
    const auto k_coo_nij = KARG(coo_nij);
    const auto k_coo_aux = KARG(coo_aux);
    const auto k_nrm = KARG(nrm);
    const auto k_rowcnt = KARG(rowcnt);
    const auto k_shard_cur = KARG(shard_cur);
    const auto k_shard_occ = KARG(shard_occ);
    const auto k_shard_cap = KARG(shard_cap);
    const auto k_cap = KARG(cap);
    const auto k_raw = KARG(raw);
    const auto k_counters = KARG(counters);
    constexpr int NIT = SLOTS_ / NW / 64;
    const int sb0 = w * (SLOTS_ / NW);
    int fj[NIT], fn[NIT], fm[NIT];
    double fs[NIT], fy[NIT], fa[NIT];
    bool fo[NIT], fk[NIT];
#pragma unroll
    for (int t = 0; t < NIT; t++) {
        const int sl = sb0 + t * 64 + lane;
        const uint32_t kj = key[sl];
        fo[t] = kj != T_EMPTY;
        fj[t] = (int)kj;
        const CM c = cm[sl];
        fn[t] = (int)(c & NMASK); fm[t] = (int)(c >> MSH);
        fs[t] = dot[sl];
        fa[t] = (ADJ && k_raw) ? dlo[sl] : 0.0;
        fy[t] = 0.0;
        if (fo[t]) {
            if (!k_raw) fy[t] = k_nrm[kj];
        }
    }
    int kept = 0, occ = 0;
#pragma unroll
    for (int t = 0; t < NIT; t++) {
        bool keep = fo[t];
        if (keep && !k_raw) {
            const double np = nx * fy[t];
            const double cs = (np != 0.0) ? 1.0 * fs[t] / np : 0.0;
            const int mn = fn[t] < k_cap ? fn[t] : k_cap;
            fs[t] = 1.0 * cs * (double)mn / (double)k_cap;
            keep = (fs[t] != 0.0) && (fm[t] != 0);
        }
        fk[t] = keep;
        kept += __popcll(__ballot(keep));
        occ += __popcll(__ballot(fo[t]));
    }
    const int shard = (blockIdx.x * NW + w) & (COO_SHARDS - 1);
    if (lane == 0 && occ) atomicAdd(&k_shard_occ[shard], (unsigned long long)occ);
    if (!kept) return;
    unsigned long long cbase = 0;
    if (lane == 0) {
        cbase = atomicAdd(&k_shard_cur[shard], (unsigned long long)kept);
        atomicAdd(&k_rowcnt[i], kept);
    }
    cbase = ((unsigned long long)(unsigned)rl32((int)(cbase >> 32), 0) << 32) | (unsigned)rl32((int)(cbase & 0xffffffffull), 0);
    if ((long long)(cbase + kept) > k_shard_cap) {
        if (lane == 0) atomicOr(&k_counters[3], 1ull);
        return;
    }
    cbase += (unsigned long long)shard * (unsigned long long)k_shard_cap;
#pragma unroll
    for (int t = 0; t < NIT; t++) {
        const unsigned long long km = __ballot(fk[t]);
        if (fk[t]) {
            const long long pp = (long long)cbase + __popcll(km & lanemask_lt());
            const int j = fj[t];
            k_coo_i[pp] = i; k_coo_j[pp] = j;
            k_coo_sim[pp] = fs[t]; k_coo_mutu[pp] = fm[t]; k_coo_nij[pp] = fn[t];
            if (k_coo_aux) k_coo_aux[pp] = fa[t];
        }
        cbase += __popcll(km);
    }
}

constexpr int HEAVY_WAVES = 4;
template <int METHOD>
__global__ __launch_bounds__(64 * HEAVY_WAVES) void k_pair_heavy(TriArgs A) {
    __shared__ uint32_t cnt[HMAX];
    __shared__ uint32_t mut[HMAX];
// ... 1154 lines not shown
    if (rcode) return rcode;
    if (I > 0)
        XM_HIP(hipMemcpy2DAsync(&h_counts[2], sizeof(int64_t), uq_ptr, sizeof(int64_t) * (size_t)I, sizeof(int64_t),
                                N_CLASSES, hipMemcpyDeviceToHost, st));
    else
        for (int c = 0; c < N_CLASSES; c++) h_counts[2 + c] = 0;
    XM_HIP(hipStreamSynchronize(st));
    h_counts[2 + N_CLASSES] = h_counts[0];
    return XMAP_OK;
}

int xmap_sim2_units(void *stream, int32_t n_items, const int64_t *item_ptr, const int32_t *Qcat, const int64_t *uq_ptr,
                    int32_t *uq_item, int32_t *uq_q, const int32_t *C, const int64_t *uc_ptr, int32_t *uc_item, int32_t *uc_c) {
    XM_ARG(item_ptr && Qcat && uq_ptr && uq_item && uq_q && C && uc_ptr && uc_item && uc_c);
    if (n_items == 0) return XMAP_OK;
    k_fill_units2<<<dim3((unsigned)(((long long)N_CLASSES * n_items + 255) / 256)), dim3(256), 0, (hipStream_t)stream>>>(
        n_items, (const long long *)item_ptr, Qcat, (const long long *)uq_ptr, uq_item, uq_q, C, (const long long *)uc_ptr, uc_item, uc_c, 0x7fffffffffffffffLL,
        0x7fffffffffffffffLL);
    XM_LAUNCH_CHECK();
    return XMAP_OK;
}

int xmap_sim3_plan(void *stream, const xmap_ratings *R, int32_t slot_target, const int64_t *pre, const int32_t *hid,
                   const int32_t *ctl, int32_t *Q, int32_t *C, uint8_t *small, uint64_t *Wp, int32_t *Qcat, int64_t *uq_ptr,
                   int64_t *uc_ptr, int32_t dups, int32_t *uq_item, int32_t *uq_q, int32_t *uc_item, int32_t *uc_c,
                   int64_t cap_light, int64_t cap_heavy, int64_t *h_out) {
    XM_SCOPE(stream);
    XM_ARG(R && Wp && pre && hid && ctl && Q && C && small && Qcat && uq_ptr && uc_ptr && h_out);
    XM_ARG(uq_item && uq_q && uc_item && uc_c && cap_light >= 0 && cap_heavy >= 0);
    XM_ARG(slot_target > 0 && slot_target <= T_SLOTS);
    hipStream_t st = (hipStream_t)stream;
    const int I = R->n_items;
    for (int c = 0; c < 10; c++) h_out[c] = 0;
    XM_HIP(hipMemsetAsync(Qcat, 0, sizeof(int32_t) * (size_t)N_CLASSES * (size_t)(I > 0 ? I : 1), st));
    if (I > 0) {
        k_plan2<<<dim3((unsigned)((I + 255) / 256)), dim3(256), 0, st>>>(
            I, (const long long *)R->item_ptr, nullptr, (const long long *)pre, (int)R->n_users + 2, hid, ctl, slot_target, dups, Q, C,
            small, (unsigned long long *)Wp, Qcat);
        XM_LAUNCH_CHECK();
    }
    int rcode = xmap_exclusive_scan_i32_to_i64(stream, Qcat, uq_ptr, (int64_t)N_CLASSES * I, nullptr);
    if (rcode) return rcode;
    rcode = xmap_exclusive_scan_i32_to_i64(stream, C, uc_ptr, I, nullptr);
    if (rcode) return rcode;
    if (I > 0) {
        k_fill_units2<<<dim3((unsigned)(((long long)N_CLASSES * I + 255) / 256)), dim3(256), 0, st>>>(
            I, (const long long *)R->item_ptr, Qcat, (const long long *)uq_ptr, uq_item, uq_q, C, (const long long *)uc_ptr, uc_item, uc_c,
            cap_light, cap_heavy);
        XM_LAUNCH_CHECK();
        XM_HIP(hipMemcpy2DAsync(&h_out[2], sizeof(int64_t), uq_ptr, sizeof(int64_t) * (size_t)I, sizeof(int64_t), N_CLASSES + 1,
                                hipMemcpyDeviceToHost, st));
        XM_HIP(hipMemcpyAsync(&h_out[1], uc_ptr + I, sizeof(int64_t), hipMemcpyDeviceToHost, st));
    }
    int32_t h_ctl[2] = {0, 0};
    XM_HIP(hipMemcpyAsync(h_ctl, ctl, 2 * sizeof(int32_t), hipMemcpyDeviceToHost, st));
    XM_HIP(hipStreamSynchronize(st));
    h_out[0] = h_out[2 + N_CLASSES];
    h_out[8] = h_ctl[0]; h_out[9] = h_ctl[1];
    if (h_ctl[1] > HMAX) {
        set_error("heavy set larger than %d", HMAX);
        return XMAP_ERR_OVERFLOW;
    }
    if (h_out[0] > cap_light || h_out[1] > cap_heavy) {
        set_error("unit arrays too small: %lld light / %lld heavy units, room for %lld / %lld", (long long)h_out[0], (long long)h_out[1],
                  (long long)cap_light, (long long)cap_heavy);
        return XMAP_ERR_CAPACITY;
    }
    return XMAP_OK;
}

int xmap_sim2_pairs(void *stream, const xmap_ratings *R, int method, int cap, const double *u_avg, const double *norms,
                    const void *rc, const void *ub, const int32_t *Q,
                    const uint8_t *small, const int32_t *uq_item, const int32_t *uq_q, const int64_t *cls_ptr ,
                    int64_t unit_lo, int64_t unit_hi, const int32_t *hid,
                    const int32_t *hlist, const int32_t *ctl, const int32_t *C, const int64_t *uc_ptr,
                    const int32_t *uc_item, const int32_t *uc_c, int32_t n_heavy_units, int32_t n_heavy, int phases,
                    double *hp_hi, double *hp_lo, int32_t *hp_cnt, int32_t *hp_mut, int64_t coo_cap, int32_t *coo_i,
                    int32_t *coo_j, double *coo_sim, int32_t *coo_mutu, int32_t *coo_nij, double *coo_ls ,
                    int32_t *rowcnt, int32_t *rowcnt_h , int64_t *d_shards ,
                    int64_t *d_counters , int32_t *mircnt ) {
    XM_SCOPE(stream);
    XM_ARG(R && u_avg && norms && rc && ub);
    XM_ARG(Q && small && uq_item && uq_q && cls_ptr && hid && hlist && ctl && C && uc_ptr && uc_item && uc_c);
    XM_ARG(coo_i && coo_j && coo_sim && coo_mutu && coo_nij && rowcnt && rowcnt_h && d_shards && d_counters);
    XM_ARG(coo_cap >= COO_SHARDS);
    XM_ARG(method == XMAP_COSINE || method == XMAP_ADJUST_COSINE || method == XMAP_COSINE_EXACT);
    XM_ARG(n_heavy_units == 0 || !(phases & 5) || (hp_hi && hp_lo && hp_cnt && hp_mut));
    hipStream_t st = (hipStream_t)stream;
    const bool exact_cos = method == XMAP_COSINE_EXACT;
    const double *nrm = norms + (method == XMAP_ADJUST_COSINE ? (size_t)R->n_items : 0);
    if (exact_cos) {
        double *zero_avg = nullptr;
        const size_t ub = sizeof(double) * (size_t)(R->n_users > 0 ? R->n_users : 1);
        XM_HIP(xm_malloc_async((void **)&zero_avg, ub, st));
        XM_HIP(hipMemsetAsync(zero_avg, 0, ub, st));
        u_avg = zero_avg;
        method = XMAP_ADJUST_COSINE;
    }
    const bool raw = (phases & 32) != 0;
    XM_ARG(!coo_ls || ((raw || method == XMAP_ADJUST_COSINE) && n_heavy_units == 0));
    XM_ARG(!raw || (coo_ls && n_heavy_units == 0 && n_heavy == 0));
    if (phases & 8) {
        XM_HIP(hipMemsetAsync(d_counters, 0, 4 * sizeof(int64_t), st));
        XM_HIP(hipMemsetAsync(d_shards, 0, 2 * COO_SHARDS * sizeof(int64_t), st));
        if (!(phases & 128)) XM_HIP(hipMemsetAsync(coo_i, 0xff, sizeof(int32_t) * (size_t)coo_cap, st));
        XM_HIP(hipMemsetAsync(rowcnt, 0, sizeof(int32_t) * (size_t)(R->n_items > 0 ? R->n_items : 1), st));
        if (mircnt) XM_HIP(hipMemsetAsync(mircnt, 0, sizeof(int32_t) * (size_t)(R->n_items > 0 ? R->n_items : 1), st));
    }
    TriArgs A;
    memset(&A, 0, sizeof(A));
    A.iptr = (const long long *)R->item_ptr; A.rc = (const RaterRec *)rc; A.ub = (const int2 *)ub;
    A.u_avg = u_avg; A.nrm = nrm; A.cap = cap;
    A.Q = Q; A.small = small; A.uq_item = uq_item; A.uq_q = uq_q; A.unit_lo = unit_lo; A.unit_hi = unit_hi;
    A.hid = hid; A.hlist = hlist; A.CH = ctl; A.uc_item = uc_item; A.uc_c = uc_c;
    A.uc_ptr = (const long long *)uc_ptr; A.C = C;
    A.hp_hi = hp_hi; A.hp_lo = hp_lo; A.hp_cnt = hp_cnt; A.hp_mut = hp_mut;
    A.shard_cap = coo_cap / COO_SHARDS; A.shard_cur = (unsigned long long *)d_shards;
    A.shard_occ = (unsigned long long *)d_shards + COO_SHARDS; A.coo_i = coo_i; A.coo_j = coo_j; A.coo_sim = coo_sim; A.coo_mutu = coo_mutu; A.coo_nij = coo_nij;
    A.coo_aux = coo_ls;
    A.raw = raw ? 1 : 0;
    A.heavy_mod = (phases >> 16) & 0xff; A.heavy_rem = (phases >> 8) & 0xff;
    if (A.heavy_mod < 1) A.heavy_mod = 1;
    A.rowcnt = rowcnt; A.mircnt = mircnt; A.rowcnt_h = rowcnt_h; A.counters = (unsigned long long *)d_counters;
    const bool heavy_aside = (phases & 7) == 7 && n_heavy_units > 0 && unit_hi > unit_lo;
    hipStream_t hs = st;
    SideStreams *side = nullptr;
    if (((phases & 2) && unit_hi > unit_lo) || heavy_aside) {
        side = side_streams();
        if (!side) return XMAP_ERR_HIP;
        XM_HIP(hipEventRecord(side->fork, st));
    }
    if (heavy_aside) {
        hs = side->s[N_CLASSES];
        XM_HIP(hipStreamWaitEvent(hs, side->fork, 0));
    }
    if ((phases & 1) && n_heavy_units > 0) {
        if (method == XMAP_COSINE) k_pair_heavy<XMAP_COSINE><<<dim3((unsigned)n_heavy_units), dim3(64 * HEAVY_WAVES), 0, hs>>>(A);
        else k_pair_heavy<XMAP_ADJUST_COSINE><<<dim3((unsigned)n_heavy_units), dim3(64 * HEAVY_WAVES), 0, hs>>>(A);
        XM_LAUNCH_CHECK();
    }
    if (heavy_aside && n_heavy > 0) {
        if (method == XMAP_COSINE) k_heavy_merge<XMAP_COSINE><<<dim3((unsigned)n_heavy), dim3(256), 0, hs>>>(A, n_heavy);
        else k_heavy_merge<XMAP_ADJUST_COSINE><<<dim3((unsigned)n_heavy), dim3(256), 0, hs>>>(A, n_heavy);
        XM_LAUNCH_CHECK();
    }
    if (heavy_aside) {
        XM_HIP(hipEventRecord(side->done[N_CLASSES], hs));
        XM_HIP(hipStreamWaitEvent(st, side->done[N_CLASSES], 0));
    }
    if ((phases & 2) && unit_hi > unit_lo) {
        for (int c = 0; c < N_CLASSES; c++) {
            const long long lo = unit_lo > cls_ptr[c] ? unit_lo : cls_ptr[c];
            const long long hi = unit_hi < cls_ptr[c + 1] ? unit_hi : cls_ptr[c + 1];
            if (hi <= lo) continue;
            A.unit_lo = lo; A.unit_hi = hi;
            const dim3 grid((unsigned)(hi - lo));
            hipStream_t cs = side->s[c];
            XM_HIP(hipStreamWaitEvent(cs, side->fork, 0));
            if (coo_ls && !raw) {
                if (c == 0) k_pair_tri<XMAP_ADJUST_COSINE, 10, 16, true><<<grid, dim3(1024), 0, cs>>>(A);
                else if (c == 1) k_pair_tri<XMAP_ADJUST_COSINE, 10, 4, true><<<grid, dim3(256), 0, cs>>>(A);
                else if (c == 2) k_pair_tri<XMAP_ADJUST_COSINE, 9, 2, true><<<grid, dim3(128), 0, cs>>>(A);
                else if (c == 3) k_pair_tri<XMAP_ADJUST_COSINE, 8, 1, true><<<grid, dim3(64), 0, cs>>>(A);
                else k_pair_tri<XMAP_ADJUST_COSINE, 7, 1, true><<<grid, dim3(64), 0, cs>>>(A);
            } else if (method == XMAP_COSINE) {
                if (c == 0) k_pair_tri<XMAP_COSINE, 10, 16, false><<<grid, dim3(1024), 0, cs>>>(A);
                else if (c == 1) k_pair_tri<XMAP_COSINE, 10, 4, false><<<grid, dim3(256), 0, cs>>>(A);
                else if (c == 2) k_pair_tri<XMAP_COSINE, 9, 2, false><<<grid, dim3(128), 0, cs>>>(A);
                else if (c == 3) k_pair_tri<XMAP_COSINE, 8, 1, false><<<grid, dim3(64), 0, cs>>>(A);
                else k_pair_tri<XMAP_COSINE, 7, 1, false><<<grid, dim3(64), 0, cs>>>(A);
            } else {
                if (c == 0) k_pair_tri<XMAP_ADJUST_COSINE, 10, 16, false><<<grid, dim3(1024), 0, cs>>>(A);
                else if (c == 1) k_pair_tri<XMAP_ADJUST_COSINE, 10, 4, false><<<grid, dim3(256), 0, cs>>>(A);
                else if (c == 2) k_pair_tri<XMAP_ADJUST_COSINE, 9, 2, false><<<grid, dim3(128), 0, cs>>>(A);
                else if (c == 3) k_pair_tri<XMAP_ADJUST_COSINE, 8, 1, false><<<grid, dim3(64), 0, cs>>>(A);
                else k_pair_tri<XMAP_ADJUST_COSINE, 7, 1, false><<<grid, dim3(64), 0, cs>>>(A);
            }
            XM_LAUNCH_CHECK();
            XM_HIP(hipEventRecord(side->done[c], cs));
            XM_HIP(hipStreamWaitEvent(st, side->done[c], 0));
        }
        A.unit_lo = unit_lo; A.unit_hi = unit_hi;
    }
    if ((phases & 4) && !heavy_aside && n_heavy_units > 0 && n_heavy > 0) {
        if (method == XMAP_COSINE) k_heavy_merge<XMAP_COSINE><<<dim3((unsigned)n_heavy), dim3(256), 0, st>>>(A, n_heavy);
        else k_heavy_merge<XMAP_ADJUST_COSINE><<<dim3((unsigned)n_heavy), dim3(256), 0, st>>>(A, n_heavy);
        XM_LAUNCH_CHECK();
    }
    if (phases & 64) {
        XM_HIP(hipMemsetAsync(d_counters + 4, 0, 2 * sizeof(int64_t), st));
        k_shard_sums<<<dim3(1), dim3(256), 0, st>>>((const unsigned long long *)d_shards, (unsigned long long *)d_counters);
        XM_LAUNCH_CHECK();
    }
    if ((phases & 16) && !raw && !mircnt && R->n_items > 0) {
        int *part = nullptr;
        XM_HIP(xm_malloc_async((void **)&part, sizeof(int) * (size_t)coo_cap, st));
        int rc16 = mirror_counts(st, R->n_items, coo_cap / COO_SHARDS, COO_SHARDS, (const unsigned long long *)d_shards, coo_i, coo_j,
                                 coo_ls != nullptr, part, rowcnt);
        if (rc16) return rc16;
    }
    return XMAP_OK;
}

int xmap_sim2_pack_partials(void *stream, int64_t n_coo, const int32_t *coo_i, const int32_t *coo_j, const double *coo_hi,
                            const double *coo_lo, const int32_t *coo_mutu, const int32_t *coo_nij, int64_t *rec ,
                            int64_t *h_count) {
    XM_SCOPE(stream);
    XM_ARG(coo_i && coo_j && coo_hi && coo_lo && coo_mutu && coo_nij && rec && h_count && n_coo >= 0);
    hipStream_t st = (hipStream_t)stream;
    unsigned long long *cur = nullptr;
    XM_HIP(xm_malloc_async((void **)&cur, sizeof(unsigned long long), st));
    XM_HIP(hipMemsetAsync(cur, 0, sizeof(unsigned long long), st));
    if (n_coo > 0) {
        k_pack_partials<<<dim3((unsigned)((n_coo + 255) / 256)), dim3(256), 0, st>>>(n_coo, coo_i, coo_j, coo_hi, coo_lo, coo_mutu,
                                                                                     coo_nij, cur, (long long *)rec);
        XM_LAUNCH_CHECK();
    }
    XM_HIP(hipMemcpyAsync(h_count, cur, sizeof(int64_t), hipMemcpyDeviceToHost, st));
    XM_HIP(hipStreamSynchronize(st));
    XM_HIP(xm_free_async(cur, st));
    return XMAP_OK;
}

// ... 75 lines not shown
        XM_LAUNCH_CHECK();
    }
    XM_HIP(hipMemcpyAsync(h_counts, cnt, 2 * sizeof(int64_t), hipMemcpyDeviceToHost, st));
    XM_HIP(hipStreamSynchronize(st));
    XM_HIP(xm_free_async(cnt, st));
    return XMAP_OK;
}

int xmap_sim2_scatter(void *stream, int32_t n_items, int64_t n_coo, const int32_t *coo_i, const int32_t *coo_j,
                      const double *coo_sim, const int32_t *coo_mutu, const int32_t *coo_nij, const double *coo_ls ,
                      const int64_t *row_ptr, int32_t *fill , const int32_t *hid, const int32_t *hlist,
                      int32_t *col, double *sim, int32_t *mutu, int32_t *nij, double *ls ) {
    XM_ARG(coo_i && coo_j && coo_sim && coo_mutu && coo_nij && row_ptr && fill && hid && hlist && col && sim && mutu && nij);
    XM_ARG((coo_ls != nullptr) == (ls != nullptr));
    hipStream_t st = (hipStream_t)stream;
    XM_HIP(hipMemsetAsync(fill, 0, sizeof(int32_t) * (size_t)(n_items > 0 ? n_items : 1), st));
    if (n_coo > 0) {
        k_scatter<<<dim3((unsigned)((n_coo + 256 * SC_U - 1) / (256 * SC_U))), dim3(256), 0, st>>>(
            n_coo, coo_i, coo_j, coo_sim, coo_mutu, coo_nij, coo_ls, (const long long *)row_ptr, fill, col, sim, mutu, nij, ls);
        XM_LAUNCH_CHECK();
    }
    return XMAP_OK;
}

int xmap_sim3_layout(void *stream, const xmap_ratings *R, int64_t *item_ptr, const double *rating64, int32_t ch_min, int32_t phases,
                     int32_t stats_lo, int32_t stats_hi, int32_t *cnt, double *u_avg, double *u_norm, int32_t *hist, int64_t *pre, int32_t *ctl, int32_t *hid, int32_t *hlist,
                     uint64_t *ub_key, void *ub, void *srec, void *bufA, void *bufB, void *rc, uint64_t *Wp, double *info,
                     double *norms, int32_t *h_ctl) {
    XM_SCOPE(stream);
    XM_ARG(R && item_ptr && (const int64_t *)item_ptr == R->item_ptr && cnt && u_avg && hist && pre && ctl && hid && hlist);
    XM_ARG(ub_key && ub && srec && bufA && bufB && rc && Wp && info && norms && ch_min >= 64);
    XM_ARG(R->nnz < 0x7fffffffLL && R->n_users < 0x7ffffff0LL && R->n_items >= 0);
    XM_ARG(rating64 || u_norm);
    XM_ARG(stats_lo >= 0 && stats_lo <= stats_hi && stats_hi <= R->n_items && (phases & ~15) == 0);
    hipStream_t st = (hipStream_t)stream;
    const int I = R->n_items;
    const long long nnz = R->nnz;
    const bool wide = rating64 != nullptr;
    const size_t In = (size_t)(I > 0 ? I : 1);
    int rcode = XMAP_OK;
    if (phases & 1) {
    XM_HIP(hipMemsetAsync(cnt, 0, sizeof(int32_t) * In, st));
    const char *cb_env = getenv("XMAP_COUNT_PART_MIN");
    const long long cb_min = cb_env ? atoll(cb_env) : 2000000ll;
    if (nnz >= cb_min && I > 0) {
        rcode = mirror_counts(st, I, nnz, 1, nullptr, nullptr, R->user_item, false, (int *)bufA, cnt);
        if (rcode) return rcode;
    } else if (nnz > 0) {
        k_count3<<<dim3((unsigned)((nnz + CNT_CHUNK - 1) / CNT_CHUNK)), dim3(256), 0, st>>>(nnz, R->user_item, cnt);
        XM_LAUNCH_CHECK();
    }
    rcode = xmap_exclusive_scan_i32_to_i64(stream, cnt, item_ptr, I, nullptr);
    if (rcode) return rcode;
    if (!wide) {
        rcode = xmap_user_stats(stream, R, u_avg, u_norm);
        if (rcode) return rcode;
    }
    const int HB = (int)R->n_users + 2;
    XM_HIP(hipMemsetAsync(hist, 0, sizeof(int32_t) * (size_t)HB, st));
    XM_HIP(hipMemsetAsync(ctl, 0x7f, sizeof(int32_t), st));
    XM_HIP(hipMemsetAsync(ctl + 1, 0, 3 * sizeof(int32_t), st));
    if (I > 0) {
        k_hist<<<dim3((unsigned)((I + 256 * HIST_PER - 1) / (256 * HIST_PER))), dim3(256), 0, st>>>(I, (const long long *)item_ptr, HB, hist);
        XM_LAUNCH_CHECK();
    }
    rcode = xmap_exclusive_scan_i32_to_i64(stream, hist, pre, HB, nullptr);
    if (rcode) return rcode;
    if (HB - 1 > ch_min) {
        k_threshold<<<dim3((unsigned)((HB + 255) / 256)), dim3(256), 0, st>>>(I, HB, (const long long *)pre, ch_min, ctl);
        XM_LAUNCH_CHECK();
    }
    if (I > 0) {
        k_mark_heavy<<<dim3((unsigned)((I + 255) / 256)), dim3(256), 0, st>>>(I, (const long long *)item_ptr, ctl, hid, hlist, ctl + 1);
        XM_LAUNCH_CHECK();
    }
    if (R->n_users > 0 && nnz > 0) {
        const dim3 grid((unsigned)((R->n_users + 15) / 16));
        if (wide)
            k_sort_profiles3<true><<<grid, dim3(256), 0, st>>>(R->n_users, (const long long *)R->user_ptr, R->user_item, nullptr, rating64,
                                                               cnt, (unsigned long long *)ub_key, ub, (unsigned long long *)srec);
        else
            k_sort_profiles3<false><<<grid, dim3(256), 0, st>>>(R->n_users, (const long long *)R->user_ptr, R->user_item, R->user_rating,
                                                                nullptr, cnt, (unsigned long long *)ub_key, ub, (unsigned long long *)srec);
        XM_LAUNCH_CHECK();
    }
    XM_HIP(hipMemsetAsync(Wp, 0, sizeof(uint64_t) * In, st));
    if (nnz > 0 && I > 0) {
        ts::Geo G;
        ts_geometry(I, nnz, wide ? ts::Chunk<3>::CH : ts::Chunk<2>::CH, G);
        rcode = ts_prepare(st, G, (const long long *)item_ptr);
        if (rcode) return rcode;
        const dim3 gridA((unsigned)((nnz + G.ch - 1) / G.ch)), gridB((unsigned)G.clist_cap), gridL((unsigned)G.slist_cap);
        if (wide) {
            ts::RecLoader<3> LA{(const unsigned long long *)srec}, LB{(const unsigned long long *)bufA};
            ts::k_ts_bin<3, false, ts::RecLoader<3>><<<gridA, dim3(ts::BT), 0, st>>>(G, LA, nnz, (unsigned long long *)bufA);
            XM_LAUNCH_CHECK();
            ts::k_ts_bin<3, true, ts::RecLoader<3>><<<gridB, dim3(ts::BT), 0, st>>>(G, LB, nnz, (unsigned long long *)bufB);
            XM_LAUNCH_CHECK();
            k_rc_tiles<true><<<dim3((unsigned)G.T), dim3(ts::CT), 0, st>>>(G, (const unsigned long long *)bufB, (const long long *)R->user_ptr,
                                                                          (ulonglong2 *)rc, (unsigned long long *)Wp);
            XM_LAUNCH_CHECK();
            k_rc_large<true><<<gridL, dim3(ts::LT), 0, st>>>(G, (const unsigned long long *)bufB, (const long long *)R->user_ptr,
                                                             (ulonglong2 *)rc, (unsigned long long *)Wp);
            XM_LAUNCH_CHECK();
        } else {
            ts::RecLoader<2> LA{(const unsigned long long *)srec}, LB{(const unsigned long long *)bufA};
            ts::k_ts_bin<2, false, ts::RecLoader<2>><<<gridA, dim3(ts::BT), 0, st>>>(G, LA, nnz, (unsigned long long *)bufA);
            XM_LAUNCH_CHECK();
            ts::k_ts_bin<2, true, ts::RecLoader<2>><<<gridB, dim3(ts::BT), 0, st>>>(G, LB, nnz, (unsigned long long *)bufB);
            XM_LAUNCH_CHECK();
            k_rc_tiles<false><<<dim3((unsigned)G.T), dim3(ts::CT), 0, st>>>(G, (const unsigned long long *)bufB, (const long long *)R->user_ptr,
                                                                           (ulonglong2 *)rc, (unsigned long long *)Wp);
            XM_LAUNCH_CHECK();
            k_rc_large<false><<<gridL, dim3(ts::LT), 0, st>>>(G, (const unsigned long long *)bufB, (const long long *)R->user_ptr,
// ... 119 lines not shown
```

x-map_amd/csrc/util.hip:

```cpp
#include <stdarg.h>
#include <stdlib.h>
#include <vector>

#include "common.h"

namespace xmap {
static thread_local char g_err[512] = "";
void set_error(const char *fmt, ...) {
    va_list ap;
    va_start(ap, fmt);
    vsnprintf(g_err, sizeof(g_err), fmt, ap);
    va_end(ap);
}

namespace {
struct Chunk { char *base; size_t size, used; };
struct Arena { int dev; hipStream_t st; std::vector<Chunk> chunks; size_t live; };
thread_local std::vector<Arena> g_arenas;
constexpr size_t ARENA_KEEP = (size_t)256 << 20;
Arena *arena_find(int dev, hipStream_t st) {
    for (Arena &a : g_arenas) if (a.dev == dev && a.st == st) return &a;
    return nullptr;
}
Arena *arena_of(hipStream_t st) {
// ... 111 lines not shown
    }
    if (threadIdx.x == 0) *grand = carry;
}

template <typename TIn>
__global__ __launch_bounds__(SCAN_THREADS) void k_tile_scan(const TIn *in, long long n, const long long *tile_off,
                                                            long long *out) {
    __shared__ long long smem[4];
    long long base = (long long)blockIdx.x * SCAN_TILE + (long long)threadIdx.x * SCAN_ITEMS;
    long long v[SCAN_ITEMS];
    long long s = 0;
#pragma unroll
    for (int k = 0; k < SCAN_ITEMS; k++) {
        v[k] = (base + k < n) ? (long long)in[base + k] : 0;
        s += v[k];
    }
    long long tot;
    long long ex = block_exclusive_scan(s, &tot, smem) + tile_off[blockIdx.x];
#pragma unroll
    for (int k = 0; k < SCAN_ITEMS; k++) {
        if (base + k < n) out[base + k] = ex;
        ex += v[k];
    }
}

template <typename TIn>
static int exclusive_scan(hipStream_t st, const TIn *in, int64_t *out, int64_t n, int64_t *h_total) {
    XM_ARG(n >= 0);
    XM_SCOPE(st);
    int64_t n_tiles = (n + SCAN_TILE - 1) / SCAN_TILE;
    long long *tile = nullptr;
    XM_HIP(xm_malloc_async((void **)&tile, sizeof(long long) * (size_t)(n_tiles + 1), st));
    if (n_tiles > 0) {
        k_tile_sums<TIn><<<dim3((unsigned)n_tiles), dim3(SCAN_THREADS), 0, st>>>(in, n, tile);
        XM_LAUNCH_CHECK();
    }
    k_scan_tile_sums<<<dim3(1), dim3(SCAN_THREADS), 0, st>>>(tile, n_tiles, (long long *)(out + n));
    XM_LAUNCH_CHECK();
    if (n_tiles > 0) {
        k_tile_scan<TIn><<<dim3((unsigned)n_tiles), dim3(SCAN_THREADS), 0, st>>>(in, n, tile, (long long *)out);
        XM_LAUNCH_CHECK();
    }
    XM_HIP(xm_free_async(tile, st));
    if (h_total) {
        XM_HIP(hipMemcpyAsync(h_total, out + n, sizeof(int64_t), hipMemcpyDeviceToHost, st));
        XM_HIP(hipStreamSynchronize(st));
    }
    return XMAP_OK;
}
}

extern "C" {
const char *xmap_last_error(void) { return xmap::g_err; }
int xmap_version(void) { return 101; }

int xmap_trim(void) {
    XM_HIP(hipDeviceSynchronize());
    int dev = 0;
    XM_HIP(hipGetDevice(&dev));
    for (xmap::Arena &a : xmap::g_arenas) {
        if (a.dev != dev || a.live != 0) continue;
        for (xmap::Chunk &c : a.chunks) (void)hipFree(c.base);
        a.chunks.clear();
    }
    return XMAP_OK;
}

int xmap_debug_arena(void *stream, int64_t *live, int64_t *reserved) {
    XM_ARG(live && reserved);
    int dev = 0;
    XM_HIP(hipGetDevice(&dev));
    *live = 0; *reserved = 0;
    if (xmap::Arena *a = xmap::arena_find(dev, (hipStream_t)stream)) {
        *live = (int64_t)a->live;
        for (xmap::Chunk &c : a->chunks) *reserved += (int64_t)c.size;
    }
    return XMAP_OK;
}
int xmap_debug_arena_call(void *stream, int64_t bytes, int fail) {
    using namespace xmap;
    XM_SCOPE(stream);
    hipStream_t st = (hipStream_t)stream;
    void *a = nullptr, *b = nullptr;
    XM_HIP(xm_malloc_async(&a, (size_t)bytes, st));
    XM_HIP(xm_malloc_async(&b, 1024, st));
    XM_ARG(!fail);
    XM_HIP(xm_free_async(b, st));
    XM_HIP(xm_free_async(a, st));
    return XMAP_OK;
}

int xmap_exclusive_scan_i64(void *stream, const int64_t *in, int64_t *out, int64_t n, int64_t *h_total) {
    return xmap::exclusive_scan<long long>((hipStream_t)stream, (const long long *)in, out, n, h_total);
}
int xmap_exclusive_scan_i32_to_i64(void *stream, const int32_t *in, int64_t *out, int64_t n, int64_t *h_total) {
    return xmap::exclusive_scan<int>((hipStream_t)stream, in, out, n, h_total);
}
}
```

x-map_amd/xmap/engine/device.py:

```python
import ctypes as C
import os

import numpy as np
import torch

from . import hipabi as abi
from .exactness import plain_sums_exact

lib = abi.lib
vp, i32, i64, check = abi.vp, abi.i32, abi.i64, abi.check


def _stream(dev):
    return C.c_void_p(torch.cuda.current_stream(dev).cuda_stream)


SLOT_TARGET = 768
CH_MIN = 2048


class DeviceRatings(object):

    def __init__(self, user_ptr, item, rating, time, n_items, attrs, device="cuda:0", rating64=False):
        self.device = torch.device(device)
# ... 319 lines not shown
        h_ctl = (C.c_int32 * 2)()
        with self.timed("tri_layout"):
            check(lib.xmap_sim2_layout(st, C.byref(R.c), vp(info), i32(ch_min), vp(L.hist), vp(L.pre), vp(L.ctl),
                                       vp(L.hid), vp(L.hlist), vp(L.ub_key), vp(L.ub), vp(L.rc), vp(L.Wp),
                                       i32(1 if dups else 0), h_ctl))
        L.CH, L.n_heavy = int(h_ctl[0]), int(h_ctl[1])
        L.slot_target = slot_target
        self._tri_plan(L, slot_target)
        both = torch.stack([L.Wp[:I].sum(), L.Wp[L.hlist[:L.n_heavy].long()].sum()]).tolist() if I else [0, 0]
        L.half_contrib, L.heavy_half = int(both[0]), int(both[1])
        return L

    def _tri_plan(self, L, slot_target):
        R = self.R
        st = _stream(self.dev)
        I = R.n_items
        L.Q = self._out(max(I, 1), torch.int32, I > 0)
        L.C = self._out(max(I, 1), torch.int32, I > 0)
        L.small = self._out(max(I, 1), torch.uint8, I > 0)
        L.Qcat = self._empty(5 * max(I, 1), torch.int32)
        L.uq_ptr = self._out(5 * I + 1, torch.int64, I > 0)
        L.uc_ptr = self._out(I + 1, torch.int64, I > 0)
        h = (C.c_int64 * 8)()
        with self.timed("tri_plan"):
            check(lib.xmap_sim2_plan(st, C.byref(R.c), i32(slot_target), vp(L.rc), vp(L.pre), vp(L.hid),
                                     vp(L.ctl), vp(L.Q), vp(L.C), vp(L.small), vp(L.Wp), vp(L.Qcat), vp(L.uq_ptr),
                                     vp(L.uc_ptr), i32(1 if getattr(L, "dups", False) else 0), h))
            L.n_light, L.n_heavy_units = int(h[0]), int(h[1])
            L.cls_ptr = (C.c_int64 * 6)(*[int(h[2 + c]) for c in range(6)])
            L.uq_item = self._empty(max(L.n_light, 1), torch.int32)
            L.uq_q = self._empty(4 * max(L.n_light, 1), torch.int32)
            L.uc_item = self._empty(max(L.n_heavy_units, 1), torch.int32)
            L.uc_c = self._empty(max(L.n_heavy_units, 1), torch.int32)
            check(lib.xmap_sim2_units(st, i32(I), vp(R.item_ptr), vp(L.Qcat), vp(L.uq_ptr), vp(L.uq_item), vp(L.uq_q),
                                      vp(L.C), vp(L.uc_ptr), vp(L.uc_item), vp(L.uc_c)))
        L.slot_target = slot_target

    def _tri_plan3(self, L, slot_target):
        R = self.R
        st = _stream(self.dev)
        I = R.n_items
        L.Q = self._out(max(I, 1), torch.int32, I > 0)
        L.C = self._out(max(I, 1), torch.int32, I > 0)
        L.small = self._out(max(I, 1), torch.uint8, I > 0)
        L.Qcat = self._empty(5 * max(I, 1), torch.int32)
        L.uq_ptr = self._out(5 * I + 1, torch.int64, I > 0)
        L.uc_ptr = self._out(I + 1, torch.int64, I > 0)
        cap_light = L.half_contrib // max(int(slot_target), 1) + I + 1
        cap_heavy = R.nnz // max(int(L.ch_min), 1) + 1025
        L.uq_item = self._empty(cap_light, torch.int32)
        L.uq_q = self._empty(4 * cap_light, torch.int32)
        L.uc_item = self._empty(cap_heavy, torch.int32)
        L.uc_c = self._empty(cap_heavy, torch.int32)
        h = (C.c_int64 * 10)()
        with self.timed("tri_plan"):
            check(lib.xmap_sim3_plan(st, C.byref(R.c), i32(slot_target), vp(L.pre), vp(L.hid), vp(L.ctl), vp(L.Q), vp(L.C),
                                     vp(L.small), vp(L.Wp), vp(L.Qcat), vp(L.uq_ptr), vp(L.uc_ptr),
                                     i32(1 if getattr(L, "dups", False) else 0), vp(L.uq_item), vp(L.uq_q), vp(L.uc_item),
                                     vp(L.uc_c), i64(cap_light), i64(cap_heavy), h))
        L.n_light, L.n_heavy_units = int(h[0]), int(h[1])
        L.cls_ptr = (C.c_int64 * 6)(*[int(h[2 + c]) for c in range(6)])
        L.CH, L.n_heavy = int(h[8]), int(h[9])
        L.slot_target = slot_target
        L.replan = self._tri_plan3

    def heavy_half(self, L):
        if getattr(L, "_heavy_half", None) is None:
            L._heavy_half = int(L.Wp[L.hlist[:L.n_heavy].long()].sum().item()) if L.n_heavy else 0
        return L._heavy_half

    def tri_pairs(self, method, cap, stats, L, unit_range=None, do_heavy=True, retry=True, rec=False, raw=False, split=False,
                  heavy_deal=None, marks=True, count_mir=False):
        R = self.R
        st = _stream(self.dev)
        m = self.pair_method(method)
        u_avg, u_norm, info, _, _ = stats
        I = R.n_items
        coo_slack = 1.0
        while True:
            lo, hi = (0, L.n_light) if unit_range is None else (int(unit_range[0]), int(unit_range[1]))
            cap_coo = (max(int(L.half_contrib * coo_slack), 1) // 4096 + 1100) * 4096
            coo_i = self._empty(cap_coo, torch.int32)
            coo_j = self._empty(cap_coo, torch.int32)
            coo_sim = self._empty(cap_coo, torch.float64)
            coo_mutu = self._empty(cap_coo, torch.int32)
            coo_nij = self._empty(cap_coo, torch.int32)
            coo_ls = self._empty(cap_coo, torch.float64) if (rec or raw) else None
            rowcnt = self._empty(max(I, 1), torch.int32)
            mircnt = self._empty(max(I, 1), torch.int32) if split else None
            nh = L.n_heavy_units if do_heavy else 0
            hp_hi = self._empty(max(nh, 1) * 1024, torch.float64)
            hp_lo = self._empty(max(nh, 1) * 1024, torch.float64)
            hp_cnt = self._empty(max(nh, 1) * 1024, torch.int32)
            hp_mut = self._empty(max(nh, 1) * 1024, torch.int32)
            d_cnt = self._zeros(6, torch.int64)
            d_shards = self._empty(2 * 4096, torch.int64)
            rowcnt_h = self._empty(64 * 1024, torch.int32)

            deal = 0 if heavy_deal is None else ((int(heavy_deal[1]) & 0xff) << 16) | ((int(heavy_deal[0]) & 0xff) << 8)

            def run(phases):
                phases |= deal | (0 if marks else 128)
                check(lib.xmap_sim2_pairs(
                    st, C.byref(R.c), m, int(cap), vp(u_avg), vp(self.norms), vp(L.rc), vp(L.ub), vp(L.Q), vp(L.small),
                    vp(L.uq_item),
                    vp(L.uq_q), L.cls_ptr, i64(lo), i64(hi), vp(L.hid), vp(L.hlist), vp(L.ctl), vp(L.C), vp(L.uc_ptr),
                    vp(L.uc_item), vp(L.uc_c), i32(nh), i32(L.n_heavy), phases,
                    vp(hp_hi), vp(hp_lo), vp(hp_cnt), vp(hp_mut), i64(cap_coo), vp(coo_i), vp(coo_j), vp(coo_sim),
                    vp(coo_mutu), vp(coo_nij), vp(coo_ls), vp(rowcnt), vp(rowcnt_h), vp(d_shards), vp(d_cnt), vp(mircnt)))
            if os.environ.get("XMAP_SPLIT_PHASES") == "1":
                with self.timed("pair_heavy"):
                    run(8 | (1 if do_heavy else 0))
                with self.timed("pair_tri"):
                    run(2 | (32 if raw else 0))
                with self.timed("heavy_merge"):
                    run((4 if do_heavy else 0) | 16)
            else:
                with self.timed("pair_tri"):
                    run(8 | 2 | 16 | 64 | (5 if do_heavy else 0) | (32 if raw else 0))
            if count_mir and split and not raw:
                with self.timed("mir_count"):
                    scratch = self._empty(cap_coo, torch.int32)
                    check(lib.xmap_sim3_mircount(st, i32(I), i64(cap_coo), vp(coo_i), vp(coo_j), vp(d_shards), i64(cap_coo),
                                                 i32(1 if rec else 0), vp(scratch), vp(mircnt)))
            h = d_cnt.tolist()
            if h[2]:
                if L.slot_target <= 32:
                    raise abi.XmapError(abi.ERR_OVERFLOW, "pair-table overflow")
                if not retry:
                    return (None, rowcnt, 0, 0) + ((None, None) if split else ()) + (1,)
                getattr(L, "replan", self._tri_plan)(L, L.slot_target // 2)
                continue
            if h[3]:
                if coo_slack > 64:
                    raise abi.XmapError(abi.ERR_CAPACITY, "half-COO overflow")
                coo_slack *= 2
                continue
            break
        if os.environ.get("XMAP_SPLIT_PHASES") == "1":
            h[4:6] = d_shards.view(2, 4096).sum(dim=1).tolist()
        n, n_unordered = int(h[4]), int(h[5])
        coo = (coo_i, coo_j, coo_sim, coo_mutu, coo_nij) + ((coo_ls,) if (rec or raw) else ())
        out = (coo, rowcnt, n, n_unordered)
        if split:
            return out + (mircnt, d_shards) + (() if retry else (0,))
        return out if retry else out + (0,)

    def tri_scatter(self, coo, rowcnt, info, n=None, L=None):
        R = self.R
        st = _stream(self.dev)
        I = R.n_items
        coo_i, coo_j, coo_sim, coo_mutu, coo_nij = [x.contiguous() for x in coo[:5]]
        coo_ls = coo[5].contiguous() if len(coo) > 5 else None
        n_scan = int(coo_i.numel())
        if n is None:
            n = n_scan
        row_ptr = self._out(I + 1, torch.int64, I > 0)
        tot = C.c_int64(0)
        check(lib.xmap_exclusive_scan_i32_to_i64(st, vp(rowcnt), vp(row_ptr), i64(I), C.byref(tot) if coo_ls is not None else None))
        kept = 2 * n if coo_ls is None else int(tot.value)
        ls = self._empty(max(kept, 1), torch.float64) if coo_ls is not None else None
        col = self._empty(max(kept, 1), torch.int32)
        sim = self._empty(max(kept, 1), torch.float64)
        mutu = self._empty(max(kept, 1), torch.int32)
        nij = self._empty(max(kept, 1), torch.int32)
        fill = self._empty(max(I, 1), torch.int32)
        with self.timed("scatter"):
          if n:
            check(lib.xmap_sim2_scatter(st, i32(I), i64(n_scan), vp(coo_i), vp(coo_j), vp(coo_sim), vp(coo_mutu),
                                        vp(coo_nij), vp(coo_ls), vp(row_ptr), vp(fill), vp(L.hid), vp(L.hlist), vp(col),
                                        vp(sim), vp(mutu), vp(nij), vp(ls)))
        S = self.sim_from_device(row_ptr, col[:kept], sim[:kept], mutu[:kept], nij[:kept], info)
        S.ls = ls[:kept] if ls is not None else None
        return S

    def rec_sim(self, cap, slot_target=SLOT_TARGET):
        R = self.R
        with self.timed("rec_stats"):
            stats, L = self.layout3(slot_target, ch_min=max(64, R.n_users + 2), wide=True)
        info = stats[2]
        if os.environ.get("XMAP_A_V2") == "1":
            coo, rowcnt, n, n_unordered = self.tri_pairs("adjust_cosine", cap, stats, L, do_heavy=False, rec=True)
            S = self.tri_scatter(coo, rowcnt, info, n, L)
        else:
            coo, own, n, n_unordered, mir, shards = self.tri_pairs("adjust_cosine", cap, stats, L, do_heavy=False, rec=True, split=True, marks=False, count_mir=True)
            S = self.tri_mirror(coo, own, mir, info, n, shards, counted=True)
        S.cap, S.n_unordered, S.layout = int(cap), n_unordered, L
        S.norm = self.norms[R.n_items:2 * R.n_items]
        return S

    def rec_select(self, S, keep):
        st = _stream(self.dev)
        I = self.R.n_items
        cnt = self._zeros(max(I, 1), torch.int32)
        col = self._empty((max(I, 1), keep), torch.int32)
        sim = self._empty((max(I, 1), keep), torch.float64)
        ls = self._empty((max(I, 1), keep), torch.float64)
        with self.timed("rec_select"):
            check(lib.xmap_rec_select(st, i32(I), vp(S.row_ptr), vp(S.col), vp(S.sim), vp(S.ls), i32(keep), vp(cnt),
                                      vp(col), vp(sim), vp(ls)))
        return cnt[:I], col[:I], sim[:I], ls[:I]

    def layout3(self, slot_target=SLOT_TARGET, ch_min=CH_MIN, wide=False, item_range=None):
        R = self.R
        st = _stream(self.dev)
        I, U, nnz = R.n_items, R.n_users, R.nnz
        n1, i1 = max(nnz, 1), max(I, 1)
        rw = 3 if wide else 2
        L = SimResult()
        cnt = self._empty(i1, torch.int32)
        u_avg = self._zeros(max(U, 1), torch.float64) if wide else self._empty(max(U, 1), torch.float64)
        u_norm = None if wide else self._empty(max(U, 1), torch.float64)
        L.hist = self._empty(U + 2, torch.int32)
        L.pre = self._empty(U + 3, torch.int64)
        L.ctl = self._empty(4, torch.int32)
        L.hid = self._empty(i1, torch.int32)
        L.hlist = self._zeros(1024, torch.int32)
        L.ub_key = self._empty(n1, torch.int64)
        L.ub = self._empty(n1 * (2 if wide else 1), torch.int64)
        srec = self._empty(n1 * rw, torch.int64)
        buf_a = self._empty(n1 * rw, torch.int64)
        buf_b = self._empty(n1 * rw, torch.int64)
        L.rc = self._empty(n1 * 2, torch.int64)
        L.Wp = self._empty(i1, torch.int64)
        L.dups = bool(wide)
        L.wide = bool(wide)
        info = self._out((i1, 4), torch.float64, I > 0)
        self.norms = self._out(2 * i1, torch.float64, I > 0)
        r64 = None
        if wide:
            r64 = R.user_rating64 if R.user_rating64 is not None else R.user_rating.double()
        def call(phases, lo, hi):
            check(lib.xmap_sim3_layout(st, C.byref(R.c), vp(R.item_ptr), vp(r64), i32(ch_min), i32(phases), i32(lo), i32(hi), vp(cnt),
                                       vp(u_avg), vp(u_norm), vp(L.hist), vp(L.pre), vp(L.ctl), vp(L.hid), vp(L.hlist),
                                       vp(L.ub_key), vp(L.ub), vp(srec), vp(buf_a), vp(buf_b), vp(L.rc), vp(L.Wp), vp(info),
                                       vp(self.norms), None))
        R.csc_ready = False
        L.ch_min = int(ch_min)
        L.half_contrib = R.half_contrib
        if item_range is None:
            with self.timed("layout3"):
                call(1 | 2 | 4, 0, I)
            self._tri_plan3(L, slot_target)
        else:
            with self.timed("layout3"):
                call(1 | 2, int(item_range[0]), int(item_range[1]))

            def finish():
                with self.timed("layout3_flags"):
                    call(4 | 8, 0, I)
                self._tri_plan3(L, slot_target)
            L.finish = finish
        return (u_avg, u_norm, info, None, None), L

    def mir_counts(self, coo, n, mir, shards=None, skip_self=False):
        I = self.R.n_items
        scratch = self._empty(max(int(n), 1), torch.int32)
        check(lib.xmap_sim3_mircount(_stream(self.dev), i32(I), i64(int(coo[0].numel())), vp(coo[0].contiguous()), vp(coo[1].contiguous()),
                                     vp(shards), i64(n), i32(1 if skip_self else 0), vp(scratch), vp(mir)))
        return mir

    def tri_mirror(self, coo, own, mir, info, n, shards=None, rows=None, counted=False):
        R = self.R
        st = _stream(self.dev)
        I = R.n_items
        coo_i, coo_j, coo_sim, coo_mutu, coo_nij = [x.contiguous() for x in coo[:5]]
        coo_ls = coo[5].contiguous() if len(coo) > 5 else None
        cap = int(coo_i.numel())
        kept = 2 * int(n)
        lo, hi = (0, I) if rows is None else (int(rows[0]), int(rows[1]))
        if rows is not None and I > 0:
            own = own.clone()
            own[:lo].zero_(); own[hi:].zero_()
            if counted:
                mir = mir.clone()
                mir[:lo].zero_(); mir[hi:].zero_()
                kept = int((own[lo:hi].long().sum() + mir[lo:hi].long().sum()).item())
        rw = 4 if coo_ls is not None else 3
        row_ptr = self._out(I + 1, torch.int64, I > 0)
        mptr = self._empty(I + 1, torch.int64)
        tot = self._empty(max(I, 1), torch.int32)
        fill = self._empty(max(I, 1), torch.int32)
        buf_a = self._empty(max(int(n), 1) * rw, torch.int64)
        buf_b = self._empty(max(int(n), 1) * rw, torch.int64)
        col = self._empty(max(kept, 1), torch.int32)
        sim = self._empty(max(kept, 1), torch.float64)
        mutu = self._empty(max(kept, 1), torch.int32)
        nij = self._empty(max(kept, 1), torch.int32)
        ls = self._empty(max(kept, 1), torch.float64) if coo_ls is not None else None
        with self.timed("scatter"):
            if not counted:
                check(lib.xmap_sim3_mircount(st, i32(I), i64(cap), vp(coo_i), vp(coo_j), vp(shards), i64(n), i32(1 if coo_ls is not None else 0),
                                             vp(buf_a), vp(mir)))
                if rows is not None and I > 0:
                    mir[:lo].zero_(); mir[hi:].zero_()
                    kept = int((own[lo:hi].long().sum() + mir[lo:hi].long().sum()).item())
            check(lib.xmap_sim3_mirror(st, i32(I), i64(cap), vp(coo_i), vp(coo_j), vp(coo_sim), vp(coo_mutu), vp(coo_nij), vp(shards), i64(n),
                                       vp(own), vp(mir), vp(tot), vp(row_ptr), vp(mptr), vp(fill), vp(buf_a), vp(buf_b), vp(col),
                                       vp(sim), vp(mutu), vp(nij), vp(coo_ls), vp(ls), i32(lo), i32(hi)))
        if coo_ls is not None:
            kept = int(row_ptr[I].item()) if I > 0 else 0
        S = self.sim_from_device(row_ptr, col[:kept], sim[:kept], mutu[:kept], nij[:kept], info)
        S.ls = ls[:kept] if ls is not None else None
        return S

    def item_sim_tri(self, method, cap, slot_target=SLOT_TARGET, ch_min=CH_MIN):
        if os.environ.get("XMAP_A_V2") == "1":
            with self.timed("stats"):
                stats = self.stats()
            L = self.tri_layout(stats, slot_target, ch_min)
            coo, rowcnt, n, n_unordered = self.tri_pairs(method, cap, stats, L)
            S = self.tri_scatter(coo, rowcnt, stats[2], n, L)
        else:
            stats, L = self.layout3(slot_target, ch_min)
            coo, rowcnt, n, n_unordered, mir, shards = self.tri_pairs(method, cap, stats, L, split=True, marks=False, count_mir=True)
            S = self.tri_mirror(coo, rowcnt, mir, stats[2], n, shards, counted=True)
        S.method = abi.METHODS[method] if isinstance(method, str) else int(method)
        S.cap = int(cap)
        S.u_avg, S.u_norm = stats[0], stats[1]
        S.n_eval, S.n_contrib = 2 * n_unordered, 2 * L.half_contrib
        S.n_units, S.layout, S.slot_target = L.n_light + L.n_heavy_units, L, L.slot_target
        return S

    def sim_from_device(self, row_ptr, col, sim, mutu, nij, info):
        S = SimResult()
        S.n_items = self.R.n_items
        n = int(col.numel())
        if n == 0:
            col = self._zeros(1, torch.int32); sim = self._zeros(1, torch.float64)
            mutu = self._zeros(1, torch.int32); nij = self._zeros(1, torch.int32)
        S.row_ptr, S.info = row_ptr.contiguous(), info
        col, sim, mutu, nij = col.contiguous(), sim.contiguous(), mutu.contiguous(), nij.contiguous()
        S.col, S.sim, S.mutu, S.nij = col[:n], sim[:n], mutu[:n], nij[:n]
        S.n_kept = n
        S.c = abi.Sim(S.n_items, S.row_ptr.data_ptr(), col.data_ptr(), sim.data_ptr(), mutu.data_ptr(),
                      nij.data_ptr(), info.data_ptr())
        S._keep = (col, sim, mutu, nij)
        return S

    def sim_from_host(self, row_ptr, col, sim, mutu, nij, info, frac=None):
        d = self.dev
        n = int(row_ptr[-1])

        def up(a, dt):
            return torch.from_numpy(np.ascontiguousarray(a if n else np.zeros(1), dt)).to(d)
        row_ptr_d = torch.from_numpy(np.ascontiguousarray(row_ptr, np.int64)).to(d)
        info_d = torch.from_numpy(np.ascontiguousarray(info, np.float64)).to(d)
        S = self.sim_from_device(row_ptr_d, up(col, np.int32)[:n], up(sim, np.float64)[:n], up(mutu, np.int32)[:n],
                                 up(nij if nij is not None else np.zeros(max(n, 1)), np.int32)[:n], info_d)
        if frac is not None:
            S.frac = up(frac, np.float64)
            S.c.frac = S.frac.data_ptr()
        return S

    def knn(self, S, top_k, bb=None, rows=None):
        R = self.R
        st = _stream(self.dev)
        I, k = R.n_items, int(top_k)
        E = ExtResult()
        E.k = k
        if bb is not None:
            E.bb = bb.to(torch.uint8).contiguous()
        else:
            E.bb = self._zeros(max(I, 1), torch.uint8)
            check(lib.xmap_bridge_flags(st, C.byref(S.c), vp(R.prefix_cls), vp(E.bb)))
        alloc = self._empty if I > 0 else self._zeros
        E.cls = alloc(max(I, 1), torch.uint8)
        E.kcnt = alloc((max(I, 1), 2), torch.int32)
        E.kcol = alloc((max(I, 1), 2, k), torch.int32)
        E.kval = alloc((max(I, 1), 2, k, 3), torch.float64)
        with self.timed("knn_classify"):
            lo, hi = (0, I) if rows is None else (int(rows[0]), int(rows[1]))
            check(lib.xmap_knn_classify(st, C.byref(S.c), k, vp(E.bb), vp(R.suffix_cls), vp(R.contains_mask),
                                        vp(E.cls), vp(E.kcnt), vp(E.kcol), vp(E.kval), i32(lo), i32(hi)))
# ... 645 lines not shown
```

x-map_amd/xmap/engine/hipabi.py:

```python
import ctypes as C
import os

HERE = os.path.dirname(os.path.abspath(__file__))
LIB_PATH = os.environ.get("XMAP_HIP_LIB") or os.path.normpath(os.path.join(HERE, "..", "..", "libxmap_hip.so"))
XLIB_PATH = os.environ.get("XMAP_HIP_XLIB") or os.path.normpath(os.path.join(HERE, "..", "..", "libxmap_hip_xcheck.so"))

COSINE, ADJUST_COSINE = 0, 1
METHODS = {"cosine": COSINE, "adjust_cosine": ADJUST_COSINE}
COSINE_EXACT = 2
TOPC = 10
MID_ROWS_SPAN = 36864
ERR_HIP, ERR_ARG, ERR_OVERFLOW, ERR_CAPACITY = -1, -2, -3, -4


class XmapError(RuntimeError):
    def __init__(self, code, msg):
        RuntimeError.__init__(self, "libxmap_hip error %d: %s" % (code, msg))
        self.code = code


class Ratings(C.Structure):
    _fields_ = [("n_users", C.c_int64), ("n_items", C.c_int32), ("nnz", C.c_int64),
                ("user_ptr", C.c_void_p), ("user_item", C.c_void_p), ("user_rating", C.c_void_p),
                ("user_time", C.c_void_p), ("item_ptr", C.c_void_p), ("item_user", C.c_void_p),
                ("item_rating", C.c_void_p), ("prefix_cls", C.c_void_p), ("suffix_cls", C.c_void_p),
                ("contains_mask", C.c_void_p), ("flags", C.c_void_p)]


class Sim(C.Structure):
    _fields_ = [("n_items", C.c_int32), ("row_ptr", C.c_void_p), ("col", C.c_void_p), ("sim", C.c_void_p),
                ("mutu", C.c_void_p), ("nij", C.c_void_p), ("info", C.c_void_p), ("frac", C.c_void_p)]


class ExtTables(C.Structure):
    _fields_ = [("n_items", C.c_int32), ("top_k", C.c_int32),
                ("cls", C.c_void_p), ("kcnt", C.c_void_p), ("kcol", C.c_void_p), ("kval", C.c_void_p), ("flags", C.c_void_p),
                ("att_ptr", C.c_void_p), ("att_idx", C.c_void_p), ("att_val", C.c_void_p),
                ("src_ptr", C.c_void_p), ("src_idx", C.c_void_p), ("src_val", C.c_void_p), ("src_flag", C.c_void_p),
                ("rnn_ptr", C.c_void_p), ("rnn_idx", C.c_void_p), ("rnn_val", C.c_void_p),
                ("n_nb", C.c_int32), ("nb_id", C.c_void_p), ("nb_list", C.c_void_p), ("midX", C.c_void_p), ("dir", C.c_void_p),
                ("dir_ptr", C.c_void_p),
                ("n_ends", C.c_int32), ("urank", C.c_void_p), ("uitem", C.c_void_p)]


class PathUnits(C.Structure):
    _fields_ = [("n_units", C.c_int32), ("unit_start", C.c_void_p), ("unit_c", C.c_void_p), ("unit_G", C.c_void_p),
                ("unit_row", C.c_void_p), ("unit_nt", C.c_void_p), ("n_heavy", C.c_int32), ("heavy_unit0", C.c_void_p)]


class PathRows(C.Structure):
    _fields_ = [("n_slots", C.c_int32), ("acc", C.c_void_p), ("touched", C.c_void_p), ("hacc", C.c_void_p),
                ("htouched", C.c_void_p)]


class PathOut(C.Structure):
    _fields_ = [("n_cand", C.c_void_p), ("top_end", C.c_void_p), ("top_val", C.c_void_p), ("xs_cap", C.c_int64),
                ("xs_off", C.c_void_p), ("xs_end", C.c_void_p), ("xs_val", C.c_void_p)]


EXPORTS = [
    "xmap_last_error", "xmap_version", "xmap_trim", "xmap_debug_arena", "xmap_debug_arena_call", "xmap_exclusive_scan_i64", "xmap_exclusive_scan_i32_to_i64",
    "xmap_build_csc", "xmap_user_stats", "xmap_item_stats", 
    "xmap_sim2_layout", "xmap_sim2_plan", "xmap_sim2_units",
    "xmap_sim2_pairs", "xmap_sim2_scatter", "xmap_sim3_layout", "xmap_sim3_plan", "xmap_sim3_mircount", "xmap_sim3_mirror", "xmap_item_partials", "xmap_item_merge", "xmap_sim2_pack_partials",
    "xmap_sim2_sort_partials", "xmap_sim2_merge_partials", "xmap_sim2_pack_pairs", "xmap_sim2_unpack_pairs", "xmap_bridge_flags", "xmap_knn_classify", "xmap_knn_thresholds", "xmap_reverse_count", "xmap_reverse_count_att_rnn",
    "xmap_reverse_fill", "xmap_topc_from_lists", "xmap_path_weights", "xmap_extend_paths", 
    "xmap_mid_rows_count", "xmap_mid_rows_place", "xmap_edge_ranges", "xmap_end_universe", "xmap_extend_cols", "xmap_extend_cols_slots", "xmap_nb_index", "xmap_path_plan", "xmap_end_order", "xmap_dense_normalize", "xmap_dense_layout", "xmap_dense_topk", "xmap_rec_select", "xmap_predict", "xmap_rec_profiles", "xmap_predict_rows", "xmap_mae", "xmap_select_map", "xmap_alterego_count", "xmap_alterego_fill",
    "xmap_feed_text", "xmap_feed_texts", "xmap_feed_merge", "xmap_feed_sizes", "xmap_feed_arrays", "xmap_feed_ids", "xmap_feed_free",
    "xmap_ctx_upload_feed", "xmap_feed_format", "xmap_ctx_create", "xmap_ctx_destroy", "xmap_ctx_upload_ratings", "xmap_ctx_item_sim", "xmap_ctx_sim_download", "xmap_ctx_extend",
    "xmap_ctx_ext_download", "xmap_ctx_ext_lists", "xmap_ctx_candidates", "xmap_ctx_generate", "xmap_ctx_gen_download",
    "xmap_ctx_rec_sim", "xmap_ctx_rec_profiles_download", "xmap_ctx_rec_download", "xmap_ctx_rec_select", "xmap_ctx_rec_set_neighbors",
    "xmap_ctx_rec_neighbors_download", "xmap_ctx_predict",
]

if not os.path.exists(LIB_PATH):
    raise ImportError("libxmap_hip.so not built (%s); the MI355X engine has no CPU fallback" % LIB_PATH)
lib = C.CDLL(LIB_PATH)
lib.xmap_last_error.restype = C.c_char_p
for _n in EXPORTS:
    getattr(lib, _n)
XCHECK_EXPORTS = ["xmap_sim_plan", "xmap_sim_units", "xmap_sim_count", "xmap_sim_fill", "xmap_sim_row_ptr", "xmap_extend_paths2",
                  "xmap_mid_tally", "xmap_mid_place"]

HEADER_PATH = os.path.normpath(os.path.join(HERE, "..", "..", "..", "include", "xmap_hip.h"))


def header_prototypes(path=HEADER_PATH):
    import re
    with open(path) as f:
        text = f.read()
    text = re.sub(r"#\s*ifdef\s+XMAP_CROSSCHECK[^\n]*\n", "\n", text)
    text = re.sub(r"/\*.*?\*/", " ", text, flags=re.S)
    text = re.sub(r"//[^\n]*", " ", text)
    out = {}
    for m in re.finditer(r"\b(?:int|void|const\s+char\s*\*)\s*(xmap_\w+)\s*\(([^;{]*?)\)\s*;", text, flags=re.S):
        name, args = m.group(1), " ".join(m.group(2).split())
        types = []
        for a in ([] if args in ("", "void") else args.split(",")):
            if "*" in a:
                types.append(C.c_void_p)
            elif "int64_t" in a:
                types.append(C.c_int64)
            elif "double" in a:
                types.append(C.c_double)
            elif "float" in a:
                types.append(C.c_float)
            else:
                types.append(C.c_int32)
        out[name] = types
    return out


PROTOTYPES = header_prototypes()


def _bind(L, names):
    for _n in names:
        _f = getattr(L, _n)
        _f.argtypes = PROTOTYPES[_n]
        if _n in ("xmap_ctx_destroy", "xmap_feed_free"):
            _f.restype = None
        elif _n != "xmap_last_error":
# ... 42 lines not shown
```

Measured before the change: 23.74 billion.

## Route adjusted-cosine pair sums through fixed-point limb atomics when exponent range allows

Adds a fixed-point accumulation path for the pair-similarity kernels. The terms are split into two 44-bit integer limbs and summed with no-return u64 LDS atomics, in place of a double-double (hi, lo) read-modify-write. The user-stats kernel now also records the min/max exponent of centred and raw ratings, and the planner uses that range to choose a summation route (plain, DD or fixed), which it reports back. A profiling microbenchmark compares claim-word DD updates against two-limb atomics. The aim is to cut the cost of contended exact accumulation, at the price of an extra exponent-scan pass and more kernel template variants.

```diff
diff --git a/include/xmap_hip.h b/include/xmap_hip.h
--- a/include/xmap_hip.h
+++ b/include/xmap_hip.h
@@ -15,6 +15,9 @@
 #define XMAP_COSINE 0
 #define XMAP_ADJUST_COSINE 1
 #define XMAP_COSINE_EXACT 2
+#define XMAP_SUM_PLAIN 0
+#define XMAP_SUM_DD 1
+#define XMAP_SUM_FIXED 2
 
 #define XMAP_TOPC 10
 
@@ -100,7 +103,10 @@
                     double *coo_ls , int32_t *rowcnt,
                     int32_t *rowcnt_h , int64_t *d_shards ,
                     int64_t *d_counters ,
-                    int32_t *mircnt );
+                    int32_t *mircnt ,
+                    int32_t x_emin, int32_t x_emax ,
+                    int32_t *h_route );
+int xmap_fx_sum(const double *terms, int64_t n, int32_t e0, int64_t *limbs , double *sum );
 int xmap_sim2_scatter(void *stream, int32_t n_items, int64_t n_coo, const int32_t *coo_i, const int32_t *coo_j,
                       const double *coo_sim, const int32_t *coo_mutu, const int32_t *coo_nij, const double *coo_ls ,
                       const int64_t *row_ptr, int32_t *fill , const int32_t *hid, const int32_t *hlist,
@@ -114,7 +120,7 @@
                      void *bufA , void *bufB , void *rc ,
                      uint64_t *Wp , double *info , double *norms , int32_t *h_ctl );
 int xmap_sim3_plan(void *stream, const xmap_ratings *R, int32_t slot_target, const int64_t *pre, const int32_t *hid,
-                   const int32_t *ctl, int32_t *Q, int32_t *C, uint8_t *small, uint64_t *Wp, int32_t *Qcat ,
+                   const int32_t *ctl , int32_t *Q, int32_t *C, uint8_t *small, uint64_t *Wp, int32_t *Qcat ,
                    int64_t *uq_ptr , int64_t *uc_ptr , int32_t dups, int32_t *uq_item, int32_t *uq_q ,
                    int32_t *uc_item, int32_t *uc_c, int64_t cap_light, int64_t cap_heavy, int64_t *h_out );
 int xmap_sim3_mircount(void *stream, int32_t n_items, int64_t coo_cap, const int32_t *coo_i, const int32_t *coo_j,
@@ -333,6 +339,7 @@
                             const float *rating, const int64_t *time, const int32_t *prefix_cls, const int32_t *suffix_cls,
                             const uint32_t *contains_mask, const uint8_t *flags);
 int xmap_ctx_item_sim(xmap_ctx *ctx, int method, int cap, int64_t *n_kept, int64_t *n_evaluated);
+int xmap_ctx_sum_route(xmap_ctx *ctx, int32_t *route);
 int xmap_ctx_sim_download(xmap_ctx *ctx, int64_t *row_ptr, int32_t *col, double *sim, int32_t *mutu, int32_t *nij, double *info,
                           double *user_avg);
 int xmap_ctx_extend(xmap_ctx *ctx, int top_k, int64_t *n_out, int64_t *n_paths);
diff --git a/profiles/lds_atomic.hip b/profiles/lds_atomic.hip
--- a/profiles/lds_atomic.hip
+++ b/profiles/lds_atomic.hip
@@ -37,6 +37,72 @@
     for (int i = threadIdx.x; i < n_slots * 4; i += 1024) chk += tab[i];
     if (chk == 12345.678) out[0] = chk;
 }
+__device__ __forceinline__ void dd_add(double &hi, double &lo, double x) {
+    double s = hi + x, bb = s - hi, e = (hi - (s - bb)) + (x - bb);
+    e += lo;
+    double h2 = s + e;
+    lo = e - (h2 - s); hi = h2;
+}
+template <int MODE, int SLOTS>
+__global__ __launch_bounds__(64, SLOTS == 128 ? 8 : 1) void k2(double *out, int steps) {
+    __shared__ unsigned long long w0[SLOTS], w1[SLOTS];
+    __shared__ unsigned short claim[MODE == 2 ? SLOTS : 1];
+    const int lane = threadIdx.x;
+    for (int i = lane; i < SLOTS; i += 64) { w0[i] = 0ull; w1[i] = 0ull; }
+    unsigned long long s = mix(blockIdx.x * 64ull + lane);
+    for (int it = 0; it < steps; it++) {
+        s = mix(s);
+        const int h = (int)(s & (SLOTS - 1));
+        const double term = ((double)((s >> 20) & 1023) - 511.5) * 0.001;
+        if (MODE == 2) {
+            typedef __attribute__((address_space(3))) volatile double lds_vf64;
+            typedef __attribute__((address_space(3))) volatile unsigned short lds_vu16;
+            lds_vf64 *vhi = (lds_vf64 *)w0, *vlo = (lds_vf64 *)w1;
+            lds_vu16 *vclaim = (lds_vu16 *)claim;
+            bool pending = true;
+            while (__ballot(pending)) {
+                if (pending) vclaim[h] = (unsigned short)lane;
+                if (pending && vclaim[h] == (unsigned short)lane) {
+                    double hi = vhi[h], lo = vlo[h];
+                    dd_add(hi, lo, term);
+                    vhi[h] = hi; vlo[h] = lo;
+                    pending = false;
+                }
+            }
+        } else {
+            const unsigned long long b = (unsigned long long)__double_as_longlong(term);
+            const int be = (int)((b >> 52) & 0x7ff);
+            const unsigned long long m = (b & 0x000fffffffffffffull) | (be ? 0x0010000000000000ull : 0ull);
+            int sh = (be ? be : 1) - 1075 + 80;
+            sh = sh < 0 ? 0 : (sh > 107 ? 107 : sh);
+            unsigned long long l0 = sh >= 44 ? 0ull : ((m << sh) & ((1ull << 44) - 1));
+            long long l1 = (long long)(sh >= 44 ? m << (sh - 44) : m >> (44 - sh));
+            if (b >> 63) { l1 = l0 ? ~l1 : -l1; l0 = (0ull - l0) & ((1ull << 44) - 1); }
+            atomicAdd(&w0[h], l0);
+            atomicAdd(&w1[h], (unsigned long long)l1);
+        }
+    }
+    __syncthreads();
+    unsigned long long chk = 0ull;
+    for (int i = lane; i < SLOTS; i += 64) chk += w0[i] ^ w1[i];
+    if (chk == 0x123456789abcdefull) out[0] = 1.0;
+}
+template <int MODE, int SLOTS>
+static int run2(double *out, hipEvent_t e0, hipEvent_t e1) {
+    const int steps = 2048, blocks = 256 * 64;
+    for (int rep = 0; rep < 2; rep++) {
+        CK(hipEventRecord(e0));
+        k2<MODE, SLOTS><<<blocks, 64>>>(out, steps);
+        CK(hipEventRecord(e1)); CK(hipEventSynchronize(e1));
+        float ms; CK(hipEventElapsedTime(&ms, e0, e1));
+        const double n = (double)blocks * 64 * steps;
+        if (rep) printf("slots %5d mode %d (%s): %7.2f ms  %.3e updates/s\n", SLOTS, MODE,
+                        MODE == 2 ? "claim-word turn, 16-B (hi, lo)" : "2 no-return u64 atomics (two limbs)", ms, n / (ms * 1e-3));
+    }
+    if (run2<2, 128>(out, e0, e1) || run2<3, 128>(out, e0, e1) || run2<2, 256>(out, e0, e1) || run2<3, 256>(out, e0, e1) ||
+        run2<2, 512>(out, e0, e1) || run2<3, 512>(out, e0, e1) || run2<2, 1024>(out, e0, e1) || run2<3, 1024>(out, e0, e1)) return 1;
+    return 0;
+}
 int main() {
     double *out; CK(hipMalloc(&out, 8));
     hipEvent_t e0, e1; CK(hipEventCreate(&e0)); CK(hipEventCreate(&e1));
@@ -55,5 +121,7 @@
                 if (rep) printf("slots %5d mode %d (%s): %7.2f ms  %.3e updates/s\n", n_slots, mode, mode ? "plain 32-B RMW" : "4 atomics + 2 two-sums", ms, n / (ms * 1e-3));
             }
     }
+    if (run2<2, 128>(out, e0, e1) || run2<3, 128>(out, e0, e1) || run2<2, 256>(out, e0, e1) || run2<3, 256>(out, e0, e1) ||
+        run2<2, 512>(out, e0, e1) || run2<3, 512>(out, e0, e1) || run2<2, 1024>(out, e0, e1) || run2<3, 1024>(out, e0, e1)) return 1;
     return 0;
 }
diff --git a/x-map_amd/csrc/api.hip b/x-map_amd/csrc/api.hip
--- a/x-map_amd/csrc/api.hip
+++ b/x-map_amd/csrc/api.hip
@@ -25,6 +25,7 @@
     xmap_ratings R;
     bool have_ratings = false;
     bool plain_exact = true;
+    int32_t sum_route = -1;
     bool have_sim = false;
     xmap_sim S;
     double *u_avg = nullptr, *u_norm = nullptr, *info = nullptr;
@@ -279,7 +280,7 @@
     int64_t *pre;
     uint64_t *ub_key, *ub, *rcrec, *Wp, *srec, *buf_a, *buf_b;
     const size_t n1 = (size_t)(nnz ? nnz : 1);
-    T_ALLOC(hist, U + 2); T_ALLOC(pre, U + 3); T_ALLOC(ctl, 4); T_ALLOC(hid, I); T_ALLOCZ(hlist, 1024);
+    T_ALLOC(hist, U + 2); T_ALLOC(pre, U + 3); T_ALLOC(ctl, 8); T_ALLOC(hid, I); T_ALLOCZ(hlist, 1024);
     T_ALLOC(ub_key, n1); T_ALLOC(ub, n1); T_ALLOC(rcrec, 2 * n1); T_ALLOC(Wp, I);
     T_ALLOC(srec, 2 * n1); T_ALLOC(buf_a, 2 * n1); T_ALLOC(buf_b, 2 * n1);
     const int ch_min = 2048;
@@ -293,7 +294,7 @@
     T_ALLOCZ(uc_ptr, I + 1);
     int slot_target = 768;
     double coo_slack = 1.0;
-    int64_t hc[10];
+    int64_t hc[14];
     int64_t n_light = 0, n_hu = 0;
     int n_heavy = 0;
     auto plan = [&](int target) -> int {
@@ -319,9 +320,11 @@
         const size_t hp = (size_t)(n_hu ? n_hu : 1) * 1024;
         T_ALLOC(hp_hi, hp); T_ALLOC(hp_lo, hp); T_ALLOC(hp_cnt, hp); T_ALLOC(hp_mut, hp);
         T_ALLOCZ(d_cnt, 6); T_ALLOC(d_shards, 2 * 4096); T_ALLOC(rowcnt_h, 64 * 1024);
+        const int xr = pair_method == XMAP_COSINE_EXACT ? 12 : 10;
         XM_TRY(xmap_sim2_pairs(c->st, &R, pair_method, cap, c->u_avg, norms, rcrec, ub, Q, small, uq_item, uq_q, hc + 2, 0, n_light, hid, hlist,
                                ctl, Cc, uc_ptr, uc_item, uc_c, (int32_t)n_hu, n_heavy, 8 | 1 | 2 | 4 | 16 | 64 | 128, hp_hi, hp_lo, hp_cnt,
-                               hp_mut, cap_coo, coo_i, coo_j, coo_sim, coo_mutu, coo_nij, nullptr, own, rowcnt_h, d_shards, d_cnt, mir));
+                               hp_mut, cap_coo, coo_i, coo_j, coo_sim, coo_mutu, coo_nij, nullptr, own, rowcnt_h, d_shards, d_cnt, mir,
+                               (int32_t)hc[xr], (int32_t)hc[xr + 1], &c->sum_route));
         int64_t h_cnt[6];
         XM_TRY(d2h(h_cnt, d_cnt, 6, c->st));
         XM_HIP(hipStreamSynchronize(c->st));
@@ -361,6 +364,12 @@
     return XMAP_OK;
 #undef T_ALLOC
 #undef T_ALLOCZ
+}
+
+int xmap_ctx_sum_route(xmap_ctx *c, int32_t *route) {
+    XM_ARG(c && route && c->have_sim);
+    *route = c->sum_route;
+    return XMAP_OK;
 }
 
 int xmap_ctx_sim_download(xmap_ctx *c, int64_t *row_ptr, int32_t *col, double *sim, int32_t *mutu, int32_t *nij, double *info,
@@ -618,7 +627,7 @@
     uint64_t *ub_key, *ub, *rcrec, *Wp, *srec, *buf_a, *buf_b;
     double *u_avg, *info, *norms;
     T_ALLOC(cnt, i1); T_ALLOCZ(u_avg, U ? U : 1); T_ALLOCZ(info, i1 * 4); T_ALLOCZ(norms, 2 * i1);
-    T_ALLOC(hist, U + 2); T_ALLOC(pre, U + 3); T_ALLOC(ctl, 4); T_ALLOC(hid, i1); T_ALLOCZ(hlist, 1024);
+    T_ALLOC(hist, U + 2); T_ALLOC(pre, U + 3); T_ALLOC(ctl, 8); T_ALLOC(hid, i1); T_ALLOCZ(hlist, 1024);
     T_ALLOC(ub_key, n1); T_ALLOC(ub, 2 * n1); T_ALLOC(rcrec, 2 * n1); T_ALLOC(Wp, i1);
     T_ALLOC(srec, 3 * n1); T_ALLOC(buf_a, 3 * n1); T_ALLOC(buf_b, 3 * n1);
     const int ch_min = (int)((U + 2 > 64) ? U + 2 : 64);
@@ -631,7 +640,7 @@
     T_ALLOCZ(uc_ptr, I + 1);
     int slot_target = 768;
     double coo_slack = 1.0;
-    int64_t hc[10];
+    int64_t hc[14];
     int64_t n_light = 0;
     auto plan = [&](int target) -> int {
         const int64_t cap_light = half_contrib / target + I + 1, cap_heavy = nnz / ch_min + 1025;
@@ -657,7 +666,7 @@
         T_ALLOCZ(d_cnt, 6); T_ALLOC(d_shards, 2 * 4096); T_ALLOC(rowcnt_h, 64 * 1024);
         XM_TRY(xmap_sim2_pairs(c->st, &P, XMAP_ADJUST_COSINE, cap, u_avg, norms, rcrec, ub, Q, small, uq_item, uq_q, hc + 2, 0, n_light, hid,
                                hlist, ctl, Cc, uc_ptr, uc_item, uc_c, 0, 0, 8 | 2 | 16 | 64 | 128, hp_hi, hp_lo, hp_cnt, hp_mut, cap_coo,
-                               coo_i, coo_j, coo_sim, coo_mutu, coo_nij, coo_ls, own, rowcnt_h, d_shards, d_cnt, mir));
+                               coo_i, coo_j, coo_sim, coo_mutu, coo_nij, coo_ls, own, rowcnt_h, d_shards, d_cnt, mir, 1, 0, nullptr));
         int64_t h_cnt[6];
         XM_TRY(d2h(h_cnt, d_cnt, 6, c->st));
         XM_HIP(hipStreamSynchronize(c->st));
diff --git a/x-map_amd/csrc/common.h b/x-map_amd/csrc/common.h
--- a/x-map_amd/csrc/common.h
+++ b/x-map_amd/csrc/common.h
@@ -44,6 +44,8 @@
 #define XM_SCOPE(stream) xmap::XmScope xm_scope_((hipStream_t)(stream))
 int radix_sort_pairs(hipStream_t st, unsigned long long *keys, int *vals, unsigned long long *keys_tmp, int *vals_tmp, long long n,
                      int bits);
+
+int user_stats(void *stream, const xmap_ratings *R, double *u_avg, double *u_norm2, int32_t *xr);
 
 constexpr int WAVE = 64;
 
diff --git a/x-map_amd/csrc/stage_a.hip b/x-map_amd/csrc/stage_a.hip
--- a/x-map_amd/csrc/stage_a.hip
+++ b/x-map_amd/csrc/stage_a.hip
@@ -11,19 +11,49 @@
 constexpr uint32_t EMPTY = 0xFFFFFFFFu;
 #endif
 
+__device__ __forceinline__ void xr_take(double x, int &lo, int &hi) {
+    const int be = (int)((__double_as_longlong(x) >> 52) & 0x7ff);
+    if (x == 0.0) return;
+    const int e = (be == 0 || be == 0x7ff) ? 0x7fffffff : be - 1023;
+    lo = e < lo ? e : lo;
+    hi = e > hi ? e : hi;
+}
 __global__ __launch_bounds__(256) void k_user_stats(long long U, const long long *ptr, const float *rating,
-                                                    double *avg, double *norm2) {
+                                                    double *avg, double *norm2, int *xr) {
     long long u = (long long)blockIdx.x * blockDim.x + threadIdx.x;
-    if (u >= U) return;
-    long long a = ptr[u], b = ptr[u + 1];
-    double s = 0.0, q = 0.0;
-    for (long long e = a; e < b; e++) {
-        double r = (double)rating[e];
-        s += r;
-        q += r * r;
-    }
-    avg[u] = (b > a) ? s / (double)(b - a) : 0.0;
-    norm2[u] = sqrt(q);
+    int lo[2] = {0x7fffffff, 0x7fffffff}, hi[2] = {-0x7fffffff, -0x7fffffff};
+    if (u < U) {
+        long long a = ptr[u], b = ptr[u + 1];
+        double s = 0.0, q = 0.0;
+        for (long long e = a; e < b; e++) {
+            double r = (double)rating[e];
+            s += r;
+            q += r * r;
+        }
+        const double av = (b > a) ? s / (double)(b - a) : 0.0;
+        avg[u] = av;
+        norm2[u] = sqrt(q);
+        if (xr)
+            for (long long e = a; e < b; e++) {
+                const double r = (double)rating[e];
+                xr_take(r - av, lo[0], hi[0]);
+                xr_take(r, lo[1], hi[1]);
+            }
+    }
+    if (!xr) return;
+#pragma unroll
+    for (int k = 0; k < 2; k++) {
+#pragma unroll
+        for (int m = 32; m >= 1; m >>= 1) {
+            const int l2 = __shfl_xor(lo[k], m, 64), h2 = __shfl_xor(hi[k], m, 64);
+            lo[k] = l2 < lo[k] ? l2 : lo[k];
+            hi[k] = h2 > hi[k] ? h2 : hi[k];
+        }
+        if (lane_id() == 0) {
+            if (lo[k] < __atomic_load_n(&xr[2 * k], __ATOMIC_RELAXED)) atomicMin(&xr[2 * k], lo[k]);
+            if (-hi[k] < __atomic_load_n(&xr[2 * k + 1], __ATOMIC_RELAXED)) atomicMin(&xr[2 * k + 1], -hi[k]);
+        }
+    }
 }
 
 constexpr int CSC_SLOTS = 4096;
@@ -389,6 +419,16 @@
 
 #endif
 
+int user_stats(void *stream, const xmap_ratings *R, double *u_avg, double *u_norm2, int32_t *xr) {
+    XM_ARG(R && u_avg && u_norm2);
+    if (R->n_users == 0) return XMAP_OK;
+    hipStream_t st = (hipStream_t)stream;
+    k_user_stats<<<dim3((unsigned)((R->n_users + 255) / 256)), dim3(256), 0, st>>>(
+        R->n_users, (const long long *)R->user_ptr, R->user_rating, u_avg, u_norm2, xr);
+    XM_LAUNCH_CHECK();
+    return XMAP_OK;
+}
+
 }
 
 using namespace xmap;
@@ -419,13 +459,7 @@
 }
 
 int xmap_user_stats(void *stream, const xmap_ratings *R, double *u_avg, double *u_norm2) {
-    XM_ARG(R && u_avg && u_norm2);
-    if (R->n_users == 0) return XMAP_OK;
-    hipStream_t st = (hipStream_t)stream;
-    k_user_stats<<<dim3((unsigned)((R->n_users + 255) / 256)), dim3(256), 0, st>>>(
-        R->n_users, (const long long *)R->user_ptr, R->user_rating, u_avg, u_norm2);
-    XM_LAUNCH_CHECK();
-    return XMAP_OK;
+    return user_stats(stream, R, u_avg, u_norm2, nullptr);
 }
 
 int xmap_item_stats(void *stream, const xmap_ratings *R, const double *u_avg, double *info, double *norms,
diff --git a/x-map_amd/csrc/stage_a2.hip b/x-map_amd/csrc/stage_a2.hip
--- a/x-map_amd/csrc/stage_a2.hip
+++ b/x-map_amd/csrc/stage_a2.hip
@@ -279,6 +279,7 @@
     int *rowcnt_h;
     unsigned long long *counters;
     int heavy_mod, heavy_rem;
+    int fx_e0;
     int raw;
 };
 
@@ -354,7 +355,39 @@
 static_assert(std::is_standard_layout<TriArgs>::value, "KARG() addresses TriArgs fields by offsetof");
 #define KARG(field) (*(decltype(TriArgs::field) const volatile __attribute__((address_space(4))) *)( \
     (const char __attribute__((address_space(4))) *)__builtin_amdgcn_kernarg_segment_ptr() + offsetof(TriArgs, field)))
-template <int METHOD, int LOG_SLOTS, int NW, bool LS>
+constexpr int FX_W = 44;
+__host__ __device__ __forceinline__ void fx_split(double term, int e0, unsigned long long &l0, long long &l1) {
+    const unsigned long long b = __builtin_bit_cast(unsigned long long, term);
+    const int be = (int)((b >> 52) & 0x7ff);
+    const unsigned long long m = (b & 0x000fffffffffffffull) | (be ? 0x0010000000000000ull : 0ull);
+    int s = (be ? be : 1) - 1075 - e0;
+    s = s < 0 ? 0 : (s > 63 + FX_W ? 63 + FX_W : s);
+    constexpr unsigned long long M0 = (1ull << FX_W) - 1;
+    l0 = s >= FX_W ? 0ull : ((m << s) & M0);
+    l1 = (long long)(s >= FX_W ? m << (s - FX_W) : m >> (FX_W - s));
+    if (b >> 63) {
+        l1 = l0 ? ~l1 : -l1;
+        l0 = (0ull - l0) & M0;
+    }
+}
+__host__ __device__ __forceinline__ double fx_round(unsigned long long limb0, long long limb1, int e0) {
+    unsigned long long lo = limb0 + ((unsigned long long)limb1 << FX_W);
+    long long hi = (limb1 >> (64 - FX_W)) + (lo < limb0 ? 1 : 0);
+    const bool neg = hi < 0;
+    if (neg) { lo = 0ull - lo; hi = ~hi + (lo == 0ull ? 1 : 0); }
+    const unsigned long long uh = (unsigned long long)hi;
+    if ((uh | lo) == 0ull) return 0.0;
+    const int lz = uh ? __builtin_clzll(uh) : 64 + __builtin_clzll(lo);
+    unsigned long long nh, nl;
+    if (lz >= 64) { nh = lo << (lz - 64); nl = 0ull; }
+    else if (lz == 0) { nh = uh; nl = lo; }
+    else { nh = (uh << lz) | (lo >> (64 - lz)); nl = lo << lz; }
+    const double d = (double)(nh | (nl ? 1ull : 0ull));
+    const double r = ldexp(d, e0 + 64 - lz);
+    return neg ? -r : r;
+}
+
+template <int METHOD, int LOG_SLOTS, int NW, bool LS, bool FIX = false>
 __global__ __launch_bounds__(64 * NW, (LOG_SLOTS == 7 && !LS) ? 8 : 1) void k_pair_tri(TriArgs A) {
     constexpr int SLOTS_ = 1 << LOG_SLOTS;
     constexpr bool ADJ = METHOD == XMAP_ADJUST_COSINE;
@@ -365,13 +398,15 @@
     constexpr uint32_t LOCKBIT = 0x80000000u;
     __shared__ uint32_t key[SLOTS_];
     __shared__ CM cm[SLOTS_];
-    __shared__ double dot[SLOTS_];
-    __shared__ double dlo[ADJ ? SLOTS_ : 1];
-    __shared__ unsigned short claim[ADJ && NW == 1 ? SLOTS_ : 1];
+    using ST = typename std::conditional<FIX, unsigned long long, double>::type;
+    __shared__ ST dot[SLOTS_];
+    __shared__ ST dlo[ADJ ? SLOTS_ : 1];
+    __shared__ unsigned short claim[ADJ && !FIX && NW == 1 ? SLOTS_ : 1];
     __shared__ double s_ny[LS ? SLOTS_ : 1];
     __shared__ unsigned long long s_ls[LS ? SLOTS_ : 1];
     __shared__ int s_ovf;
     static_assert(!LS || ADJ, "the local-sensitivity pass keeps the similarity in dlo[]");
+    static_assert(!FIX || (ADJ && !LS), "fixed-point sums: the adjusted-cosine instantiations of stage A");
 
     const int lane = lane_id();
     const long long unit = A.unit_lo + blockIdx.x;
@@ -381,14 +416,15 @@
     const int q = uniform(ud.x), p0 = uniform(ud.y), p1 = uniform(ud.z), Qi = uniform(ud.w);
     const int w = uniform((int)uniform((int)(threadIdx.x >> 6)));
     for (int s = threadIdx.x; s < SLOTS_; s += 64 * NW) {
-        key[s] = T_EMPTY; cm[s] = (CM)0; dot[s] = 0.0;
-        if (ADJ) dlo[s] = 0.0;
+        key[s] = T_EMPTY; cm[s] = (CM)0; dot[s] = (ST)0;
+        if (ADJ) dlo[s] = (ST)0;
     }
     if (NW > 1) {
         if (threadIdx.x == 0) s_ovf = 0;
         __syncthreads();
     }
     const double nx = A.nrm[i];
+    const int fx_e0 = FIX ? A.fx_e0 : 0;
     int ovf = 0;
 
     constexpr int RB = (NW == 1 || NW == 16) ? 64 : 16;
@@ -481,9 +517,17 @@
         if (act) {
             const CM inc = (CM)1 | (((((unsigned)jw) >> 31) == gei) ? ((CM)1 << MSH) : (CM)0);
             atomicAdd(&cm[h], inc);
-            if (METHOD == XMAP_COSINE) atomicAdd(&dot[h], (1.0 * ri) * (double)rj);
-        }
-        if (ADJ) {
+            if constexpr (METHOD == XMAP_COSINE) atomicAdd(&dot[h], (1.0 * ri) * (double)rj);
+        }
+        if constexpr (FIX) {
+            const double term = (ri - a) * ((double)rj - a);
+            unsigned long long l0; long long l1;
+            fx_split(term, fx_e0, l0, l1);
+            if (act && term != 0.0) {
+                atomicAdd(&dot[h], l0);
+                atomicAdd(&dlo[h], (unsigned long long)l1);
+            }
+        } else if constexpr (ADJ) {
             const double term = (ri - a) * ((double)rj - a);
             typedef __attribute__((address_space(3))) volatile double lds_vf64;
             typedef __attribute__((address_space(3))) volatile unsigned short lds_vu16;
@@ -529,13 +573,13 @@
             const uint32_t kj = key[s];
             if (kj == T_EMPTY) continue;
             int n = (int)(cm[s] & NMASK);
-            double inner = dot[s];
+            double inner = (double)dot[s];
             if ((int)kj == i) { n *= 2; inner *= 2.0; }
             const double ny = A.nrm[kj];
             const double np = nx * ny;
             cm[s] = (CM)(unsigned)n;
-            dot[s] = inner;
-            dlo[s] = weighted((np != 0.0) ? 1.0 * inner / np : 0.0, n, A.cap);
+            dot[s] = (ST)inner;
+            dlo[s] = (ST) weighted((np != 0.0) ? 1.0 * inner / np : 0.0, n, A.cap);
             s_ny[s] = ny;
             s_ls[s] = 0ull;
         }
@@ -601,8 +645,13 @@
         fj[t] = (int)kj;
         const CM c = cm[sl];
         fn[t] = (int)(c & NMASK); fm[t] = (int)(c >> MSH);
-        fs[t] = dot[sl];
-        fa[t] = (ADJ && k_raw) ? dlo[sl] : 0.0;
+        if constexpr (FIX) {
+            fs[t] = fx_round(dot[sl], (long long)dlo[sl], fx_e0);
+            fa[t] = 0.0;
+        } else {
+            fs[t] = dot[sl];
+            fa[t] = (ADJ && k_raw) ? dlo[sl] : 0.0;
+        }
         fy[t] = 0.0;
         if (fo[t]) {
             if (!k_raw) fy[t] = k_nrm[kj];
@@ -1863,11 +1912,12 @@
                                 hipMemcpyDeviceToHost, st));
         XM_HIP(hipMemcpyAsync(&h_out[1], uc_ptr + I, sizeof(int64_t), hipMemcpyDeviceToHost, st));
     }
-    int32_t h_ctl[2] = {0, 0};
-    XM_HIP(hipMemcpyAsync(h_ctl, ctl, 2 * sizeof(int32_t), hipMemcpyDeviceToHost, st));
+    int32_t h_ctl[8] = {0, 0, 0, 0, 0, 0, 0, 0};
+    XM_HIP(hipMemcpyAsync(h_ctl, ctl, 8 * sizeof(int32_t), hipMemcpyDeviceToHost, st));
     XM_HIP(hipStreamSynchronize(st));
     h_out[0] = h_out[2 + N_CLASSES];
     h_out[8] = h_ctl[0]; h_out[9] = h_ctl[1];
+    for (int k = 0; k < 4; k++) h_out[10 + k] = (k & 1) ? -(int64_t)h_ctl[4 + k] : (int64_t)h_ctl[4 + k];
     if (h_ctl[1] > HMAX) {
         set_error("heavy set larger than %d", HMAX);
         return XMAP_ERR_OVERFLOW;
@@ -1877,6 +1927,32 @@
                   (long long)cap_light, (long long)cap_heavy);
         return XMAP_ERR_CAPACITY;
     }
+    return XMAP_OK;
+}
+
+static bool fx_route(int emin, int emax, long long n_terms, int *e0) {
+    const char *force = getenv("XMAP_ADJ_DD");
+    if (force && force[0] == '1') return false;
+    if (emin > emax || emin < -500 || emax > 500) return false;
+    int lg = 0;
+    while (lg < 62 && (1ll << lg) < n_terms) lg++;
+    if (FX_W + lg > 64) return false;
+    if (2 * (emax - emin) + 54 - FX_W + lg > 63) return false;
+    *e0 = 2 * emin - 52;
+    return true;
+}
+
+int xmap_fx_sum(const double *terms, int64_t n, int32_t e0, int64_t *limbs, double *sum) {
+    XM_ARG((terms || n == 0) && n >= 0 && limbs && sum);
+    unsigned long long l0 = 0ull;
+    long long l1 = 0;
+    for (int64_t k = 0; k < n; k++) {
+        unsigned long long a; long long b;
+        fx_split(terms[k], e0, a, b);
+        if (terms[k] != 0.0) { l0 += a; l1 = (long long)((unsigned long long)l1 + (unsigned long long)b); }
+    }
+    limbs[0] = (int64_t)l0; limbs[1] = l1;
+    *sum = fx_round(l0, l1, e0);
     return XMAP_OK;
 }
 
@@ -1889,7 +1965,8 @@
                     double *hp_hi, double *hp_lo, int32_t *hp_cnt, int32_t *hp_mut, int64_t coo_cap, int32_t *coo_i,
                     int32_t *coo_j, double *coo_sim, int32_t *coo_mutu, int32_t *coo_nij, double *coo_ls ,
                     int32_t *rowcnt, int32_t *rowcnt_h , int64_t *d_shards ,
-                    int64_t *d_counters , int32_t *mircnt ) {
+                    int64_t *d_counters , int32_t *mircnt , int32_t x_emin, int32_t x_emax,
+                    int32_t *h_route ) {
     XM_SCOPE(stream);
     XM_ARG(R && u_avg && norms && rc && ub);
     XM_ARG(Q && small && uq_item && uq_q && cls_ptr && hid && hlist && ctl && C && uc_ptr && uc_item && uc_c);
@@ -1909,6 +1986,9 @@
         method = XMAP_ADJUST_COSINE;
     }
     const bool raw = (phases & 32) != 0;
+    int fx_e0 = 0;
+    const bool fix = method == XMAP_ADJUST_COSINE && !raw && !coo_ls && fx_route(x_emin, x_emax, R->n_users, &fx_e0);
+    if (h_route) *h_route = method == XMAP_COSINE ? XMAP_SUM_PLAIN : (fix ? XMAP_SUM_FIXED : XMAP_SUM_DD);
     XM_ARG(!coo_ls || ((raw || method == XMAP_ADJUST_COSINE) && n_heavy_units == 0));
     XM_ARG(!raw || (coo_ls && n_heavy_units == 0 && n_heavy == 0));
     if (phases & 8) {
@@ -1930,6 +2010,7 @@
     A.shard_occ = (unsigned long long *)d_shards + COO_SHARDS; A.coo_i = coo_i; A.coo_j = coo_j; A.coo_sim = coo_sim; A.coo_mutu = coo_mutu; A.coo_nij = coo_nij;
     A.coo_aux = coo_ls;
     A.raw = raw ? 1 : 0;
+    A.fx_e0 = fx_e0;
     A.heavy_mod = (phases >> 16) & 0xff; A.heavy_rem = (phases >> 8) & 0xff;
     if (A.heavy_mod < 1) A.heavy_mod = 1;
     A.rowcnt = rowcnt; A.mircnt = mircnt; A.rowcnt_h = rowcnt_h; A.counters = (unsigned long long *)d_counters;
@@ -1980,6 +2061,12 @@
                 else if (c == 2) k_pair_tri<XMAP_COSINE, 9, 2, false><<<grid, dim3(128), 0, cs>>>(A);
                 else if (c == 3) k_pair_tri<XMAP_COSINE, 8, 1, false><<<grid, dim3(64), 0, cs>>>(A);
                 else k_pair_tri<XMAP_COSINE, 7, 1, false><<<grid, dim3(64), 0, cs>>>(A);
+            } else if (fix) {
+                if (c == 0) k_pair_tri<XMAP_ADJUST_COSINE, 10, 16, false, true><<<grid, dim3(1024), 0, cs>>>(A);
+                else if (c == 1) k_pair_tri<XMAP_ADJUST_COSINE, 10, 4, false, true><<<grid, dim3(256), 0, cs>>>(A);
+                else if (c == 2) k_pair_tri<XMAP_ADJUST_COSINE, 9, 2, false, true><<<grid, dim3(128), 0, cs>>>(A);
+                else if (c == 3) k_pair_tri<XMAP_ADJUST_COSINE, 8, 1, false, true><<<grid, dim3(64), 0, cs>>>(A);
+                else k_pair_tri<XMAP_ADJUST_COSINE, 7, 1, false, true><<<grid, dim3(64), 0, cs>>>(A);
             } else {
                 if (c == 0) k_pair_tri<XMAP_ADJUST_COSINE, 10, 16, false><<<grid, dim3(1024), 0, cs>>>(A);
                 else if (c == 1) k_pair_tri<XMAP_ADJUST_COSINE, 10, 4, false><<<grid, dim3(256), 0, cs>>>(A);
@@ -2161,14 +2248,14 @@
     }
     rcode = xmap_exclusive_scan_i32_to_i64(stream, cnt, item_ptr, I, nullptr);
     if (rcode) return rcode;
+    XM_HIP(hipMemsetAsync(ctl, 0x7f, 8 * sizeof(int32_t), st));
+    XM_HIP(hipMemsetAsync(ctl + 1, 0, 3 * sizeof(int32_t), st));
     if (!wide) {
-        rcode = xmap_user_stats(stream, R, u_avg, u_norm);
+        rcode = user_stats(stream, R, u_avg, u_norm, ctl + 4);
         if (rcode) return rcode;
     }
     const int HB = (int)R->n_users + 2;
     XM_HIP(hipMemsetAsync(hist, 0, sizeof(int32_t) * (size_t)HB, st));
-    XM_HIP(hipMemsetAsync(ctl, 0x7f, sizeof(int32_t), st));
-    XM_HIP(hipMemsetAsync(ctl + 1, 0, 3 * sizeof(int32_t), st));
     if (I > 0) {
         k_hist<<<dim3((unsigned)((I + 256 * HIST_PER - 1) / (256 * HIST_PER))), dim3(256), 0, st>>>(I, (const long long *)item_ptr, HB, hist);
         XM_LAUNCH_CHECK();
diff --git a/x-map_amd/csrc/util.hip b/x-map_amd/csrc/util.hip
--- a/x-map_amd/csrc/util.hip
+++ b/x-map_amd/csrc/util.hip
@@ -187,7 +187,7 @@
 
 extern "C" {
 const char *xmap_last_error(void) { return xmap::g_err; }
-int xmap_version(void) { return 101; }
+int xmap_version(void) { return 102; }
 
 int xmap_trim(void) {
     XM_HIP(hipDeviceSynchronize());
diff --git a/x-map_amd/xmap/engine/device.py b/x-map_amd/xmap/engine/device.py
--- a/x-map_amd/xmap/engine/device.py
+++ b/x-map_amd/xmap/engine/device.py
@@ -395,7 +395,7 @@
         L.uq_q = self._empty(4 * cap_light, torch.int32)
         L.uc_item = self._empty(cap_heavy, torch.int32)
         L.uc_c = self._empty(cap_heavy, torch.int32)
-        h = (C.c_int64 * 10)()
+        h = (C.c_int64 * 14)()
         with self.timed("tri_plan"):
             check(lib.xmap_sim3_plan(st, C.byref(R.c), i32(slot_target), vp(L.pre), vp(L.hid), vp(L.ctl), vp(L.Q), vp(L.C),
                                      vp(L.small), vp(L.Wp), vp(L.Qcat), vp(L.uq_ptr), vp(L.uc_ptr),
@@ -404,6 +404,7 @@
         L.n_light, L.n_heavy_units = int(h[0]), int(h[1])
         L.cls_ptr = (C.c_int64 * 6)(*[int(h[2 + c]) for c in range(6)])
         L.CH, L.n_heavy = int(h[8]), int(h[9])
+        L.x_range = {abi.ADJUST_COSINE: (int(h[10]), int(h[11])), abi.COSINE_EXACT: (int(h[12]), int(h[13]))}
         L.slot_target = slot_target
         L.replan = self._tri_plan3
 
@@ -441,6 +442,8 @@
             rowcnt_h = self._empty(64 * 1024, torch.int32)
 
             deal = 0 if heavy_deal is None else ((int(heavy_deal[1]) & 0xff) << 16) | ((int(heavy_deal[0]) & 0xff) << 8)
+            x_lo, x_hi = getattr(L, "x_range", {}).get(m, (1, 0))
+            route = C.c_int32(-1)
 
             def run(phases):
                 phases |= deal | (0 if marks else 128)
@@ -450,7 +453,8 @@
                     vp(L.uq_q), L.cls_ptr, i64(lo), i64(hi), vp(L.hid), vp(L.hlist), vp(L.ctl), vp(L.C), vp(L.uc_ptr),
                     vp(L.uc_item), vp(L.uc_c), i32(nh), i32(L.n_heavy), phases,
                     vp(hp_hi), vp(hp_lo), vp(hp_cnt), vp(hp_mut), i64(cap_coo), vp(coo_i), vp(coo_j), vp(coo_sim),
-                    vp(coo_mutu), vp(coo_nij), vp(coo_ls), vp(rowcnt), vp(rowcnt_h), vp(d_shards), vp(d_cnt), vp(mircnt)))
+                    vp(coo_mutu), vp(coo_nij), vp(coo_ls), vp(rowcnt), vp(rowcnt_h), vp(d_shards), vp(d_cnt), vp(mircnt),
+                    i32(x_lo), i32(x_hi), C.byref(route)))
             if os.environ.get("XMAP_SPLIT_PHASES") == "1":
                 with self.timed("pair_heavy"):
                     run(8 | (1 if do_heavy else 0))
@@ -483,6 +487,7 @@
         if os.environ.get("XMAP_SPLIT_PHASES") == "1":
             h[4:6] = d_shards.view(2, 4096).sum(dim=1).tolist()
         n, n_unordered = int(h[4]), int(h[5])
+        L.sum_route = int(route.value)
         coo = (coo_i, coo_j, coo_sim, coo_mutu, coo_nij) + ((coo_ls,) if (rec or raw) else ())
         out = (coo, rowcnt, n, n_unordered)
         if split:
@@ -556,7 +561,7 @@
         u_norm = None if wide else self._empty(max(U, 1), torch.float64)
         L.hist = self._empty(U + 2, torch.int32)
         L.pre = self._empty(U + 3, torch.int64)
-        L.ctl = self._empty(4, torch.int32)
+        L.ctl = self._empty(8, torch.int32)
         L.hid = self._empty(i1, torch.int32)
         L.hlist = self._zeros(1024, torch.int32)
         L.ub_key = self._empty(n1, torch.int64)
@@ -663,6 +668,7 @@
         S.u_avg, S.u_norm = stats[0], stats[1]
         S.n_eval, S.n_contrib = 2 * n_unordered, 2 * L.half_contrib
         S.n_units, S.layout, S.slot_target = L.n_light + L.n_heavy_units, L, L.slot_target
+        S.sum_route = L.sum_route
         return S
 
     def sim_from_device(self, row_ptr, col, sim, mutu, nij, info):
diff --git a/x-map_amd/xmap/engine/hipabi.py b/x-map_amd/xmap/engine/hipabi.py
--- a/x-map_amd/xmap/engine/hipabi.py
+++ b/x-map_amd/xmap/engine/hipabi.py
@@ -8,6 +8,7 @@
 COSINE, ADJUST_COSINE = 0, 1
 METHODS = {"cosine": COSINE, "adjust_cosine": ADJUST_COSINE}
 COSINE_EXACT = 2
+SUM_PLAIN, SUM_DD, SUM_FIXED = 0, 1, 2
 TOPC = 10
 MID_ROWS_SPAN = 36864
 ERR_HIP, ERR_ARG, ERR_OVERFLOW, ERR_CAPACITY = -1, -2, -3, -4
@@ -62,12 +63,12 @@
     "xmap_last_error", "xmap_version", "xmap_trim", "xmap_debug_arena", "xmap_debug_arena_call", "xmap_exclusive_scan_i64", "xmap_exclusive_scan_i32_to_i64",
     "xmap_build_csc", "xmap_user_stats", "xmap_item_stats", 
     "xmap_sim2_layout", "xmap_sim2_plan", "xmap_sim2_units",
-    "xmap_sim2_pairs", "xmap_sim2_scatter", "xmap_sim3_layout", "xmap_sim3_plan", "xmap_sim3_mircount", "xmap_sim3_mirror", "xmap_item_partials", "xmap_item_merge", "xmap_sim2_pack_partials",
+    "xmap_sim2_pairs", "xmap_fx_sum", "xmap_sim2_scatter", "xmap_sim3_layout", "xmap_sim3_plan", "xmap_sim3_mircount", "xmap_sim3_mirror", "xmap_item_partials", "xmap_item_merge", "xmap_sim2_pack_partials",
     "xmap_sim2_sort_partials", "xmap_sim2_merge_partials", "xmap_sim2_pack_pairs", "xmap_sim2_unpack_pairs", "xmap_bridge_flags", "xmap_knn_classify", "xmap_knn_thresholds", "xmap_reverse_count", "xmap_reverse_count_att_rnn",
     "xmap_reverse_fill", "xmap_topc_from_lists", "xmap_path_weights", "xmap_extend_paths", 
     "xmap_mid_rows_count", "xmap_mid_rows_place", "xmap_edge_ranges", "xmap_end_universe", "xmap_extend_cols", "xmap_extend_cols_slots", "xmap_nb_index", "xmap_path_plan", "xmap_end_order", "xmap_dense_normalize", "xmap_dense_layout", "xmap_dense_topk", "xmap_rec_select", "xmap_predict", "xmap_rec_profiles", "xmap_predict_rows", "xmap_mae", "xmap_select_map", "xmap_alterego_count", "xmap_alterego_fill",
     "xmap_feed_text", "xmap_feed_texts", "xmap_feed_merge", "xmap_feed_sizes", "xmap_feed_arrays", "xmap_feed_ids", "xmap_feed_free",
-    "xmap_ctx_upload_feed", "xmap_feed_format", "xmap_ctx_create", "xmap_ctx_destroy", "xmap_ctx_upload_ratings", "xmap_ctx_item_sim", "xmap_ctx_sim_download", "xmap_ctx_extend",
+    "xmap_ctx_upload_feed", "xmap_feed_format", "xmap_ctx_create", "xmap_ctx_destroy", "xmap_ctx_upload_ratings", "xmap_ctx_item_sim", "xmap_ctx_sum_route", "xmap_ctx_sim_download", "xmap_ctx_extend",
     "xmap_ctx_ext_download", "xmap_ctx_ext_lists", "xmap_ctx_candidates", "xmap_ctx_generate", "xmap_ctx_gen_download",
     "xmap_ctx_rec_sim", "xmap_ctx_rec_profiles_download", "xmap_ctx_rec_download", "xmap_ctx_rec_select", "xmap_ctx_rec_set_neighbors",
     "xmap_ctx_rec_neighbors_download", "xmap_ctx_predict",
```

Result: slower. 23.35 billion (-1.6%).
